# muyeon-jo/POI_recommendation_models

Hardware: AMD Instinct MI355X
Metric: scored (user,POI) pairs/sec full-catalog + top-50, 100k POIs (higher is better)
Workload: dtype fp32-faithful: W1 x products as 6 f16 MFMA products of exact hi/mid/lo fp16 splits (dropped terms <= ~2^-33 relative, below fp32 rounding), fp32 accumulate; all other arithmetic fp32

## Files before the change

### include/nais.h

```cpp
#ifndef NAIS_H_
#define NAIS_H_

#include <stddef.h>
#include <stdint.h>

#ifdef __cplusplus
extern "C" {
#endif

#define NAIS_ABI_VERSION 19

#define NAIS_VARIANT_BASIC 0
#define NAIS_VARIANT_REGION 1
#define NAIS_VARIANT_REGION_DISTANCE 2
#define NAIS_VARIANT_DISTANCE 3

#define NAIS_PRECISION_FP32 0
#define NAIS_PRECISION_FP16X3 1
#define NAIS_PRECISION_FP16X3_PAIRSPLIT 2
#define NAIS_PRECISION_FP16X6 3
#define NAIS_PRECISION_FP16X6_PAIRSPLIT 4

#define NAIS_FLAG_SIGMOID 1

#define NAIS_OK 0
#define NAIS_E_INVALID (-1)
#define NAIS_E_UNSUPPORTED (-2)
#define NAIS_E_HIP (-3)
#define NAIS_E_WORKSPACE (-4)

typedef struct nais_params {
  int32_t variant;
  int32_t embed_dim;
  int32_t item_dim;
  int32_t region_dim;
  int32_t hidden;
  int32_t din;
  int64_t num_pois;
  int64_t num_regions;
  float beta;
  int32_t precision;
  const float* embed_history;
  const float* embed_target;
  const float* embed_region;
  const float* w1;
  const float* b1;
  const float* w2;
  const float* dist_w;
  const float* dist_b;
} nais_params_t;

typedef struct nais_prior {
  double a, b, alpha;
  const double* coords;
} nais_prior_t;

int32_t nais_abi_version(void);

const char* nais_last_error(void);

int32_t nais_forward(const nais_params_t* params,
                     const int64_t* hist, int64_t b, int64_t n, int64_t hist_ld,
                     const int64_t* target,
                     const int64_t* hist_region, int64_t hist_region_ld,
                     const int64_t* target_region,
                     const float* target_lat_long, int64_t latlon_ld,
                     float* out, int32_t* nan_count, int32_t flags, void* stream);

size_t nais_score_topk_workspace_size(const nais_params_t* params, int32_t num_users, int32_t k,
                                      int32_t with_prior);
int32_t nais_score_topk(const nais_params_t* params,
                        const int64_t* indptr, const int64_t* indices,
                        const int32_t* users, int32_t num_users, int32_t k,
                        const int64_t* region_of, const double* coords,
                        const double* latlon_mat, const nais_prior_t* prior,
                        int32_t* out_ids, float* out_scores,
                        int32_t* nan_count, int32_t* short_count,
                        void* workspace, size_t workspace_bytes, void* stream);

int32_t nais_score_catalog(const nais_params_t* params,
                           const int64_t* indptr, const int64_t* indices,
                           const int32_t* users, int32_t num_users,
                           const int64_t* region_of, const double* coords, const double* latlon_mat,
                           float* scores, int64_t score_ld, int32_t* nan_count, void* stream);

int32_t nais_powerlaw_prior(const double* coords, int64_t num_pois, const int64_t* indptr,
                            const int64_t* indices, const int32_t* users, int32_t num_users, double a,
                            double b, double* out, int64_t out_ld, double* out_max, void* stream);

int32_t nais_distance_histogram(const double* coords, const int64_t* indptr, const int64_t* indices,
                                int64_t num_users, uint64_t* hist, int64_t nbins, uint64_t* overflow,
                                void* stream);

int32_t nais_topk_rows(const float* scores, int64_t score_ld, int64_t num_pois, int32_t num_rows,
                       int32_t k, int32_t* out_ids, float* out_scores, int32_t* short_count,
                       void* stream);

int32_t nais_gather_rows(const float* table, int64_t rows, int32_t dim,
                         const int64_t* idx, int64_t m, float* out, void* stream);

size_t nais_pair_rows_workspace_size(int64_t num_pois);
int32_t nais_pair_rows(const int64_t* indptr, const int64_t* indices, const int32_t* users,
                       int32_t num_users, int64_t num_pois, int32_t* rowmap, int64_t* items,
                       int64_t* num_items, void* workspace, size_t workspace_bytes, void* stream);
int32_t nais_pair_table(const nais_params_t* params, const int64_t* items, int64_t num_items,
                        int64_t col0, int64_t cols, const int64_t* region_of,
                        const double* coords, const double* latlon_mat, float* e, float* es,
                        int64_t ld, int32_t* work, void* stream);
int32_t nais_pair_gather(const float* e, const float* es, int64_t ld, const int32_t* rowmap,
                         const int64_t* indptr, const int64_t* indices, const int32_t* users,
                         int32_t num_users, int64_t col0, int64_t cols, float beta, float* scores,
                         int64_t score_ld, int64_t score_col0, int32_t* nan_count, void* stream);
int32_t nais_pair_gather_topk(const float* e, const float* es, int64_t ld, const int32_t* rowmap,
                              const int64_t* indptr, const int64_t* indices, const int32_t* users,
                              int32_t num_users, int64_t col0, int64_t cols, float beta, int32_t k,
                              uint64_t* keys, int32_t* kcount, int32_t* nan_count, int32_t* work,
                              void* stream);
int32_t nais_topk_keys_finish(const uint64_t* keys, const int32_t* kcount, int32_t num_users, int32_t k,
                              int32_t* out_ids, float* out_scores, int32_t* short_count, void* stream);
int32_t nais_pair_table_split(const nais_params_t* params, const int64_t* items, int64_t num_items,
                              int64_t col0, int64_t cols, const int64_t* region_of,
                              const double* coords, const double* latlon_mat, uint32_t* hi,
                              uint32_t* ex, int64_t ld, int32_t* work, void* stream);
int32_t nais_pair_bound_topk(const uint32_t* hi, int64_t ld, const int32_t* rowmap,
                             const int64_t* indptr, const int64_t* indices, const int32_t* users,
                             int32_t num_users, int64_t col0, int64_t cols, float beta, int32_t k,
                             uint64_t* lo_keys, int32_t* lo_count, uint64_t* surv, int32_t* surv_count,
                             int32_t surv_cap, const int32_t* entry_rows, const int64_t* spans,
                             int32_t* work, void* stream);
int32_t nais_pair_refine_topk(const uint32_t* ex, int64_t block_stride,
                              int64_t ld, int64_t block_cols, const int32_t* rowmap,
                              const int64_t* indptr, const int64_t* indices, const int32_t* users,
                              int32_t num_users, int64_t col0, int64_t cols, float beta, int32_t k,
                              const uint64_t* lo_keys, const int32_t* lo_count, const uint64_t* surv,
                              const int32_t* surv_count, int32_t surv_cap, const uint64_t* tau,
                              uint64_t* keys, int32_t* kcount, int32_t* nan_count, int32_t* stats,
                              const int32_t* entry_rows, void* stream);
int32_t nais_pair_table_bound(const nais_params_t* params, const int64_t* items, int64_t num_items,
                              int64_t col0, int64_t cols, const int64_t* region_of,
                              const double* coords, const double* latlon_mat, uint32_t* hi,
                              int64_t ld, void* stream);
int32_t nais_pair_table_bound_queued(const nais_params_t* params, const int64_t* items,
                                     int64_t num_items, int64_t col0, int64_t cols,
                                     const int64_t* region_of, const double* coords,
                                     const double* latlon_mat, uint32_t* hi, int64_t ld,
                                     int32_t* work, void* stream);
int32_t nais_pair_table_bound1_queued(const nais_params_t* params, const int64_t* items,
                                      int64_t num_items, int64_t col0, int64_t cols,
                                      const int64_t* region_of, const double* coords,
                                      const double* latlon_mat, uint32_t* hi, int64_t ld,
                                      int32_t* work, void* stream);
int32_t nais_pair_bound_topk_widened(const uint32_t* hi, int64_t ld, const int32_t* rowmap,
                                     const int64_t* indptr, const int64_t* indices, const int32_t* users,
                                     int32_t num_users, int64_t col0, int64_t cols, float beta, int32_t k,
                                     uint64_t* lo_keys, int32_t* lo_count, uint64_t* surv,
                                     int32_t* surv_count, int32_t surv_cap, const int32_t* entry_rows,
                                     const int64_t* spans, const float* widen, int32_t* work,
                                     void* stream);
int32_t nais_pair_scales(const nais_params_t* params, const int64_t* items, int64_t num_items,
                         int64_t col0, int64_t cols, int64_t block_cols, float* row_scales,
                         float* col_scales, void* stream);
int32_t nais_pair_refine_topk_exact(const nais_params_t* params, const float* row_scales,
                                    const float* col_scales, const int32_t* rowmap, const int64_t* indptr,
                                    const int64_t* indices, const int32_t* users, int32_t num_users,
                                    int64_t col0, int64_t cols, int32_t k, const uint64_t* lo_keys,
                                    const int32_t* lo_count, const uint64_t* surv, const int32_t* surv_count,
                                    int32_t surv_cap, const uint64_t* tau, uint64_t* keys, int32_t* kcount,
                                    int32_t* nan_count, int32_t* stats, const int32_t* entry_rows,
                                    void* stream);
int32_t nais_pair_recompute(const nais_params_t* params, const int64_t* items, int64_t num_items,
                            const float* row_scales, const float* col_scales, int64_t col0, int64_t cols,
                            const int32_t* rows, int64_t num_rows, const int64_t* columns,
                            int64_t num_columns, float* out_e, float* out_es, void* stream);
int32_t nais_pair_prior_table(const double* coords, int64_t num_pois, const int64_t* items,
                              int64_t num_items, int64_t col0, int64_t cols, double a, double b,
                              double* pr, int64_t ld, void* stream);
#define NAIS_PRIOR_FINITE 1
int32_t nais_pair_prior_gather(const double* pr, int64_t ld, const int32_t* rowmap,
                               const int64_t* indptr, const int64_t* indices, const int32_t* users,
                               int32_t num_users, int64_t col0, int64_t cols, double* g, int64_t g_ld,
                               int64_t g_col0, uint64_t* gmax_bits, int32_t flags, void* stream);
int32_t nais_topk_blend_rows(const float* scores, int64_t score_ld, const double* g, int64_t g_ld,
                             const uint64_t* gmax_bits, int64_t num_pois, int32_t num_rows, int32_t k,
                             double alpha, int32_t* out_ids, float* out_scores, int32_t* short_count,
                             void* stream);
int32_t nais_topk_blend_rows_f64(const float* scores, int64_t score_ld, const double* g, int64_t g_ld,
                                 const uint64_t* gmax_bits, int64_t num_pois, int32_t num_rows, int32_t k,
                                 double alpha, int32_t* out_ids, float* out_scores, double* out_blend,
                                 int32_t* short_count, void* stream);
int32_t nais_topk_merge_f64(const double* keys, const int64_t* ids, int32_t num_rows, int32_t m,
                            int32_t k, int64_t* out_ids, float* out_scores, double* out_keys,
                            void* stream);

int32_t nais_stream_create_cu_mask(const uint32_t* cu_mask, uint32_t mask_words, void** stream);
int32_t nais_stream_destroy(void* stream);

int32_t nais_new4_tables(const float* embed_history, const float* embed_target,
                         const float* embed_ingoing, const float* embed_outgoing,
                         int64_t num_pois, int32_t embed_size, const int64_t* near_pois,
                         int32_t num_near, float* ext_history, float* ext_target, void* stream);

int32_t nais_near_attention(const float* query_src, const float* kv_src, int64_t num_pois,
                            int32_t dim, const int64_t* near_pois, int32_t num_near,
                            const float* wq, const float* bq, const float* wk, const float* bk,
                            const float* wv, const float* bv, float scale_dim, float* out,
                            int64_t out_ld, void* stream);
int32_t nais_copy_columns(const float* src, int64_t src_ld, int64_t rows, int32_t dim, float* dst,
                          int64_t dst_ld, int32_t dst_col0, void* stream);

typedef struct nais_dot_tables {
  int32_t embed_dim;
  int64_t num_pois;
  float beta;
  float scale_dim;
  const float* xh;
  const float* xt;
  const float* qt;
  const float* kh;
  const float* vh;
} nais_dot_tables_t;
// ... 194 lines not shown
```

### poi_recommendation_models_amd/_capi.py

```python
from __future__ import annotations

import ctypes
import os

HERE = os.path.dirname(os.path.abspath(__file__))
LIB_NAME = "libnais_hip.so"
LIB_PATH = os.path.join(HERE, LIB_NAME)

ABI_VERSION = 19
PRECISION_FP32, PRECISION_FP16X3, PRECISION_FP16X3_PAIRSPLIT = 0, 1, 2
PRIOR_FINITE = 1
PRECISION_FP16X6, PRECISION_FP16X6_PAIRSPLIT = 3, 4
VARIANT_BASIC, VARIANT_REGION, VARIANT_REGION_DISTANCE, VARIANT_DISTANCE = 0, 1, 2, 3
FLAG_SIGMOID = 1

EXPORTS = ("nais_abi_version", "nais_last_error", "nais_forward", "nais_score_topk_workspace_size",
           "nais_score_topk", "nais_score_catalog", "nais_topk_rows", "nais_powerlaw_prior",
           "nais_distance_histogram", "nais_gather_rows", "nais_train_workspace_size",
           "nais_train_forward", "nais_train_backward", "nais_dropout_mask", "nais_adagrad",
           "nais_adagrad_rows", "nais_train_step_workspace_size", "nais_train_step", "nais_train_step_ex",
           "nais_make_train_batch", "nais_new4_tables", "nais_pair_rows_workspace_size",
           "nais_pair_rows", "nais_pair_table", "nais_pair_gather", "nais_stream_create_cu_mask",
           "nais_stream_destroy", "nais_near_attention", "nais_copy_columns",
           "nais_linear_rows", "nais_dot_forward", "nais_dot_pair_table", "nais_dot_single_fixup",
           "nais_disent_forward", "nais_pair_distances", "nais_train_forward_ex",
           "nais_train_backward_ex", "nais_pair_gather_topk", "nais_topk_keys_finish",
           "nais_pair_prior_table",
           "nais_pair_prior_gather", "nais_topk_blend_rows", "nais_topk_blend_rows_f64",
           "nais_topk_merge_f64", "nais_train_ucache_size", "nais_pair_table_split",
           "nais_pair_bound_topk", "nais_pair_refine_topk", "nais_pair_table_bound",
           "nais_pair_bound_topk_widened", "nais_pair_scales", "nais_pair_refine_topk_exact",
           "nais_pair_recompute", "nais_pair_table_bound_queued", "nais_pair_table_bound1_queued",
           "nais_geoie_table", "nais_geoie_score", "nais_geoie_forward",
           "nais_geoie_make_train_batch", "nais_geoie_train_step_workspace_size",
           "nais_geoie_train_step", "nais_sgd")


class NaisGeoIEParams(ctypes.Structure):
    _fields_ = [("embed_dim", ctypes.c_int32), ("num_users", ctypes.c_int64),
                ("num_pois", ctypes.c_int64), ("a", ctypes.c_float), ("b", ctypes.c_float)] + \
        [(n, ctypes.c_void_p) for n in ("user_pref", "poi_pref", "geo_influence", "geo_suscept")]


class NaisGeoIETrainGrads(ctypes.Structure):
    _fields_ = [(n, ctypes.c_void_p) for n in ("user_pref", "poi_pref", "geo_suscept", "geo_influence")]


class NaisDotTables(ctypes.Structure):
    _fields_ = [("embed_dim", ctypes.c_int32), ("num_pois", ctypes.c_int64), ("beta", ctypes.c_float),
                ("scale_dim", ctypes.c_float), ("xh", ctypes.c_void_p), ("xt", ctypes.c_void_p),
                ("qt", ctypes.c_void_p), ("kh", ctypes.c_void_p), ("vh", ctypes.c_void_p)]


class NaisTrainSide(ctypes.Structure):
    _fields_ = [("hist_region", ctypes.c_void_p), ("target_region", ctypes.c_void_p),
                ("target_lat_long", ctypes.c_void_p), ("latlon_ld", ctypes.c_int64),
                ("ucache", ctypes.c_void_p), ("ucache_bytes", ctypes.c_uint64)]


class NaisTrainGrads(ctypes.Structure):
    _fields_ = [(n, ctypes.c_void_p) for n in ("embed_history", "embed_target", "embed_region", "w1",
                                               "b1", "w2", "dist_w", "dist_b")]


class NaisDisentParams(ctypes.Structure):
    _fields_ = [("embed_dim", ctypes.c_int32), ("hidden", ctypes.c_int32), ("num_pois", ctypes.c_int64),
                ("num_regions", ctypes.c_int64), ("beta", ctypes.c_float)] + \
        [(n, ctypes.c_void_p) for n in ("embed_history", "embed_target", "embed_region", "embed_distance",
                                        "w1", "b1", "w2", "region_w1", "region_b1", "region_w2")]


class NaisParams(ctypes.Structure):
    _fields_ = [
        ("variant", ctypes.c_int32), ("embed_dim", ctypes.c_int32), ("item_dim", ctypes.c_int32),
        ("region_dim", ctypes.c_int32), ("hidden", ctypes.c_int32), ("din", ctypes.c_int32),
        ("num_pois", ctypes.c_int64), ("num_regions", ctypes.c_int64),
        ("beta", ctypes.c_float), ("precision", ctypes.c_int32),
        ("embed_history", ctypes.c_void_p), ("embed_target", ctypes.c_void_p),
        ("embed_region", ctypes.c_void_p), ("w1", ctypes.c_void_p), ("b1", ctypes.c_void_p),
        ("w2", ctypes.c_void_p), ("dist_w", ctypes.c_void_p), ("dist_b", ctypes.c_void_p),
    ]


class NaisPrior(ctypes.Structure):
    _fields_ = [("a", ctypes.c_double), ("b", ctypes.c_double), ("alpha", ctypes.c_double),
                ("coords", ctypes.c_void_p)]


class NaisAdagradState(ctypes.Structure):
    _fields_ = [("lr", ctypes.c_float), ("lr_decay", ctypes.c_float),
                ("weight_decay", ctypes.c_float), ("eps", ctypes.c_float), ("step", ctypes.c_int64)] + \
        [(n, ctypes.c_void_p) for n in ("sum_embed_history", "sum_embed_target", "sum_w1", "sum_b1",
                                        "sum_w2", "grad_embed_history", "grad_embed_target",
                                        "grad_small", "stamp_embed_history", "stamp_embed_target")]


class NaisAdagradSide(ctypes.Structure):
    _fields_ = [(n, ctypes.c_void_p) for n in ("sum_embed_region", "grad_embed_region", "sum_dist_w",
                                               "sum_dist_b", "grad_dist")]


class NaisError(RuntimeError):
    pass


_lib = None


def load(path: str | None = None):
    global _lib
    if _lib is not None and path is None:
        return _lib
    p = path or os.environ.get("NAIS_HIP_LIB", LIB_PATH)
    if not os.path.exists(p):
        raise NaisError(f"{p} not found: build it with `python -c 'import __graft_entry__ as g; g.build()'` "
# ... 48 lines not shown
    lib.nais_train_step.argtypes = [ctypes.POINTER(NaisParams), ctypes.POINTER(NaisAdagradState), vp,
                                    i64, vp, vp, i64, f32, u64, vp, vp, vp, vp, sz, vp]
    lib.nais_train_step_ex.restype = i32
    lib.nais_train_step_ex.argtypes = [ctypes.POINTER(NaisParams), ctypes.POINTER(NaisTrainSide),
                                       ctypes.POINTER(NaisAdagradState), ctypes.POINTER(NaisAdagradSide),
                                       vp, i64, vp, vp, i64, f32, u64, vp, vp, vp, vp, sz, vp]
    lib.nais_make_train_batch.restype = i32
    lib.nais_make_train_batch.argtypes = [vp, vp, i64, i64, i64, i32, u64, vp, vp, vp, vp, vp]
    lib.nais_new4_tables.restype = i32
    lib.nais_new4_tables.argtypes = [vp, vp, vp, vp, i64, i32, vp, i32, vp, vp, vp]
    lib.nais_near_attention.restype = i32
    lib.nais_near_attention.argtypes = [vp, vp, i64, i32, vp, i32, vp, vp, vp, vp, vp, vp,
                                        ctypes.c_float, vp, i64, vp]
    lib.nais_linear_rows.restype = i32
    lib.nais_linear_rows.argtypes = [vp, i64, i64, i32, vp, vp, i32, vp, i64, vp]
    lib.nais_dot_forward.restype = i32
    lib.nais_dot_forward.argtypes = [ctypes.POINTER(NaisDotTables), vp, i64, i64, i64, vp, vp, vp, i32, vp]
    lib.nais_dot_pair_table.restype = i32
    lib.nais_dot_pair_table.argtypes = [ctypes.POINTER(NaisDotTables), vp, i64, i64, i64, vp, vp, i64, vp]
    lib.nais_dot_single_fixup.restype = i32
    lib.nais_dot_single_fixup.argtypes = [ctypes.POINTER(NaisDotTables), vp, vp, vp, i64, i64, i64, vp,
                                          i64, i64, vp]
    lib.nais_train_forward_ex.restype = i32
    lib.nais_train_forward_ex.argtypes = [ctypes.POINTER(NaisParams), ctypes.POINTER(NaisTrainSide), vp, i64,
                                          vp, i64, f32, u64, vp, vp, vp, vp, ctypes.c_size_t, vp]
    lib.nais_train_backward_ex.restype = i32
    lib.nais_train_backward_ex.argtypes = [ctypes.POINTER(NaisParams), ctypes.POINTER(NaisTrainSide), vp,
                                           i64, vp, i64, f32, u64, vp, vp, vp,
                                           ctypes.POINTER(NaisTrainGrads), vp, ctypes.c_size_t, vp]
    lib.nais_disent_forward.restype = i32
    lib.nais_disent_forward.argtypes = [ctypes.POINTER(NaisDisentParams), vp, i64, i64, i64, vp, vp, i64, vp,
                                        vp, i64, vp, vp, i32, vp]
    lib.nais_pair_distances.restype = i32
    lib.nais_pair_distances.argtypes = [vp, vp, i64, vp, i64, vp, vp]
    lib.nais_copy_columns.restype = i32
    lib.nais_copy_columns.argtypes = [vp, i64, i64, i32, vp, i64, i32, vp]
    lib.nais_pair_rows_workspace_size.restype = sz
    lib.nais_pair_rows_workspace_size.argtypes = [i64]
    lib.nais_pair_rows.restype = i32
    lib.nais_pair_rows.argtypes = [vp, vp, vp, i32, i64, vp, vp, vp, vp, sz, vp]
    lib.nais_pair_table.restype = i32
    lib.nais_pair_table.argtypes = [ctypes.POINTER(NaisParams), vp, i64, i64, i64, vp, vp, vp, vp, vp,
                                    i64, vp, vp]
    lib.nais_pair_gather.restype = i32
    lib.nais_pair_gather.argtypes = [vp, vp, i64, vp, vp, vp, vp, i32, i64, i64, f32, vp, i64, i64, vp,
                                     vp]
    lib.nais_pair_gather_topk.restype = i32
    lib.nais_pair_gather_topk.argtypes = [vp, vp, i64, vp, vp, vp, vp, i32, i64, i64, f32, i32, vp, vp, vp,
                                          vp, vp]
    lib.nais_pair_prior_table.restype = i32
    lib.nais_pair_prior_table.argtypes = [vp, i64, vp, i64, i64, i64, f64, f64, vp, i64, vp]
    lib.nais_pair_prior_gather.restype = i32
    lib.nais_pair_prior_gather.argtypes = [vp, i64, vp, vp, vp, vp, i32, i64, i64, vp, i64, i64, vp, i32, vp]
    lib.nais_topk_blend_rows.restype = i32
    lib.nais_topk_blend_rows.argtypes = [vp, i64, vp, i64, vp, i64, i32, i32, f64, vp, vp, vp, vp]
    lib.nais_topk_blend_rows_f64.restype = i32
    lib.nais_topk_blend_rows_f64.argtypes = [vp, i64, vp, i64, vp, i64, i32, i32, f64, vp, vp, vp, vp, vp]
    lib.nais_train_ucache_size.restype = sz
    lib.nais_train_ucache_size.argtypes = [ctypes.POINTER(NaisParams), i64, i64]
    lib.nais_topk_merge_f64.restype = i32
    lib.nais_topk_merge_f64.argtypes = [vp, vp, i32, i32, i32, vp, vp, vp, vp]
    lib.nais_topk_keys_finish.restype = i32
    lib.nais_topk_keys_finish.argtypes = [vp, vp, i32, i32, vp, vp, vp, vp]
    lib.nais_pair_table_split.restype = i32
    lib.nais_pair_table_split.argtypes = [ctypes.POINTER(NaisParams), vp, i64, i64, i64, vp, vp, vp, vp,
                                          vp, i64, vp, vp]
    lib.nais_pair_bound_topk.restype = i32
    lib.nais_pair_bound_topk.argtypes = [vp, i64, vp, vp, vp, vp, i32, i64, i64, f32, i32, vp, vp, vp, vp,
                                         i32, vp, vp, vp, vp]
    lib.nais_pair_refine_topk.restype = i32
    lib.nais_pair_refine_topk.argtypes = [vp, i64, i64, i64, vp, vp, vp, vp, i32, i64, i64, f32, i32,
                                          vp, vp, vp, vp, i32, vp, vp, vp, vp, vp, vp, vp]
    lib.nais_pair_table_bound.restype = i32
    lib.nais_pair_table_bound.argtypes = [ctypes.POINTER(NaisParams), vp, i64, i64, i64, vp, vp, vp, vp,
                                          i64, vp]
    lib.nais_pair_table_bound_queued.restype = i32
    lib.nais_pair_table_bound_queued.argtypes = [ctypes.POINTER(NaisParams), vp, i64, i64, i64, vp, vp, vp,
                                                 vp, i64, vp, vp]
    lib.nais_pair_table_bound1_queued.restype = i32
    lib.nais_pair_table_bound1_queued.argtypes = lib.nais_pair_table_bound_queued.argtypes
    lib.nais_pair_bound_topk_widened.restype = i32
    lib.nais_pair_bound_topk_widened.argtypes = [vp, i64, vp, vp, vp, vp, i32, i64, i64, f32, i32, vp, vp,
                                                 vp, vp, i32, vp, vp, vp, vp, vp]
    lib.nais_pair_scales.restype = i32
    lib.nais_pair_scales.argtypes = [ctypes.POINTER(NaisParams), vp, i64, i64, i64, i64, vp, vp, vp]
    lib.nais_pair_refine_topk_exact.restype = i32
    lib.nais_pair_refine_topk_exact.argtypes = [ctypes.POINTER(NaisParams), vp, vp, vp, vp, vp, vp, i32,
                                                i64, i64, i32, vp, vp, vp, vp, i32, vp, vp, vp, vp, vp,
                                                vp, vp]
    lib.nais_pair_recompute.restype = i32
    lib.nais_pair_recompute.argtypes = [ctypes.POINTER(NaisParams), vp, i64, vp, vp, i64, i64, vp, i64,
                                        vp, i64, vp, vp, vp]
    lib.nais_geoie_table.restype = i32
    lib.nais_geoie_table.argtypes = [vp, vp, i64, vp, i64, i64, i64, f32, f32, vp, i64, vp]
    lib.nais_geoie_score.restype = i32
    lib.nais_geoie_score.argtypes = [ctypes.POINTER(NaisGeoIEParams), vp, vp, vp, i32, vp, vp, i64,
                                     i64, i64, i64, vp, i64, i64, vp, vp]
    lib.nais_geoie_forward.restype = i32
    lib.nais_geoie_forward.argtypes = [ctypes.POINTER(NaisGeoIEParams), vp, vp, vp, i64, i64, i64, vp,
                                       i64, vp, vp]
    lib.nais_geoie_make_train_batch.restype = i32
    lib.nais_geoie_make_train_batch.argtypes = [vp, vp, vp, i64, i64, i64, i32, u64, vp, vp, vp, vp, vp,
                                                vp, vp, i64, vp, vp]
    lib.nais_geoie_train_step_workspace_size.restype = sz
    lib.nais_geoie_train_step_workspace_size.argtypes = [ctypes.POINTER(NaisGeoIEParams), i64, i64]
    lib.nais_geoie_train_step.restype = i32
    lib.nais_geoie_train_step.argtypes = [ctypes.POINTER(NaisGeoIEParams), i64, vp, i64, vp, vp, vp, i64,
                                          vp, i64, f32, f32, vp, vp, i32, vp, vp, vp, vp,
                                          ctypes.POINTER(NaisGeoIETrainGrads), vp, sz, vp]
    lib.nais_sgd.restype = i32
    lib.nais_sgd.argtypes = [vp, vp, i64, i32, f32, f32, vp, i32, i64, vp, vp]
    lib.nais_stream_create_cu_mask.restype = i32
    lib.nais_stream_create_cu_mask.argtypes = [vp, ctypes.c_uint32, ctypes.POINTER(ctypes.c_void_p)]
    lib.nais_stream_destroy.restype = i32
    lib.nais_stream_destroy.argtypes = [vp]
    v = lib.nais_abi_version()
    if v != ABI_VERSION:
        raise NaisError(f"{p}: ABI version {v}, expected {ABI_VERSION}")
    if path is None:
        _lib = lib
    return lib


def check(rc: int, what: str):
    if rc != 0:
        msg = load().nais_last_error().decode(errors="replace")
        raise NaisError(f"{what} failed ({rc}): {msg}")


def ptr(t) -> int | None:
    return None if t is None else t.data_ptr()


def stream_handle(device) -> int:
    import torch
    return torch.cuda.current_stream(device).cuda_stream
```

### poi_recommendation_models_amd/catalog.py

```python
from __future__ import annotations

import ctypes
import os

import numpy as np
import torch

from . import _capi


class DeviceCSR:

    def __init__(self, train_matrix, device):
        X = train_matrix.tocsr() if not hasattr(train_matrix, "indptr") else train_matrix
        if not X.has_sorted_indices:
            X = X.sorted_indices()
        self.shape = X.shape
        self.host_indptr = np.asarray(X.indptr, dtype=np.int64)
        self.host_indices = np.asarray(X.indices, dtype=np.int64)
        self.hist_len = np.diff(self.host_indptr)
        self.indptr = torch.from_numpy(self.host_indptr).to(device)
        self.indices = torch.from_numpy(self.host_indices).to(device)
        self.device = device
        self.key = (id(train_matrix), X.shape, X.nnz)
# ... 92 lines not shown
    if stream is not None:
        ext = torch.cuda.ExternalStream(stream, device=dev)
        cur = torch.cuda.current_stream(dev)
        ext.wait_stream(cur)
        with torch.cuda.stream(ext):
            out = score_topk(model, train_matrix, users, k, region_of, coords, latlon_mat, ordered,
                             None, prior, strategy, _on_caller_stream=True)
        cur.wait_stream(ext)
        for t in out:
            t.record_stream(cur)
        return out
    strategy = strategy or getattr(model, "catalog_strategy", "auto")
    if strategy not in ("auto", "direct", "pairs"):
        raise ValueError(f"unknown strategy {strategy!r}")
    if model._pairs_only:
        if prior is not None:
            raise NotImplementedError(f"{type(model).__name__}: no power-law prior on its catalog path")
        strategy = "pairs"
    if strategy != "direct":
        got = _score_topk_pairs(model, train_matrix, users, k, region_of, coords, latlon_mat,
                                stream, force=strategy == "pairs", prior=prior,
                                no_side_streams=_on_caller_stream)
        if got is not None:
            return got
    csr = device_csr(train_matrix, dev)
    P = model._item_tables()[0].shape[0]
    if csr.shape[1] != P:
        raise ValueError(f"train_matrix has {csr.shape[1]} POIs, model has {P}")
    users = _user_array(users)
    if len(users) == 0:
        return (torch.empty(0, k, dtype=torch.int64, device=dev),
                torch.empty(0, k, dtype=torch.float32, device=dev))
    if np.any(P - csr.hist_len[users] < k):
        raise RuntimeError("selected index k out of range")
    order = lpt_order(users, csr.hist_len, P) if ordered else users
    u_dev = torch.from_numpy(order.astype(np.int32)).to(dev)
    reg, cor, llm = _side_inputs(model, dev, region_of, coords, latlon_mat)
    n = len(order)
    ids = torch.empty(n, k, dtype=torch.int32, device=dev)
    sc = torch.empty(n, k, dtype=torch.float32, device=dev)
    counters = torch.zeros(2, dtype=torch.int32, device=dev)
    lib = _capi.load()
    prm = model._score_params()
    pri, pri_coords = None, None
    if prior is not None:
        pa, pb, alpha, pc = prior
        pri_coords = torch.as_tensor(np.ascontiguousarray(pc, dtype=np.float64)).to(dev)
        prior_flags = _capi.PRIOR_FINITE if _prior_entries_finite(pa, pb) else 0
        pri = _capi.NaisPrior(float(pa), float(pb), float(alpha), pri_coords.data_ptr())
    nbytes = lib.nais_score_topk_workspace_size(prm, n, k, int(prior is not None))
    ws = _workspace(dev, nbytes)
    st = stream if stream is not None else _capi.stream_handle(dev)
    rc = lib.nais_score_topk(prm, csr.indptr.data_ptr(), csr.indices.data_ptr(), u_dev.data_ptr(),
                             n, k, _capi.ptr(reg), _capi.ptr(cor), _capi.ptr(llm),
                             None if pri is None else ctypes.byref(pri),
                             ids.data_ptr(), sc.data_ptr(), counters[0:1].data_ptr(),
                             counters[1:2].data_ptr(), ws.data_ptr(), ws.numel(), st)
    _capi.check(rc, "nais_score_topk")
    model._last_nan = counters[0:1]
    if ordered:
        inv = np.empty(n, dtype=np.int64)
        pos = {int(u): i for i, u in enumerate(order)}
        inv[:] = [pos[int(u)] for u in users]
        inv_t = torch.from_numpy(inv).to(dev)
        ids, sc = ids.index_select(0, inv_t), sc.index_select(0, inv_t)
    return ids.to(torch.int64), sc


PAIR_BLOCK_COLS = 512
PAIR_TABLE_CUS = -1
PAIR_FIRST_TABLE_ALL_CUS = True
PAIR_FUSED_TOPK = True
PAIR_LPT_ORDER = True
PAIR_STRIPE = 256
PAIR_CU_LAYOUT = "contiguous"
PAIR_TABLE_GATHER_FRAC = 0.0
PAIR_TABLE_STREAMS = int(os.environ.get("NAIS_PAIR_TABLE_STREAMS", "2"))
PAIR_WORK_QUEUE = os.environ.get("NAIS_PAIR_WORK_QUEUE", "1") != "0"
PAIR_SPLIT_STEP = 8
X3Q_RATE = 1.10e15
X3Q_GATHER_MARGIN = 1.14
X1Q_RATE = 6.0e14
X1Q_GATHER_MARGIN = 1.34
PAIR_BOUNDED = True
PAIR_ONDEMAND_REFINE = os.environ.get("NAIS_PAIR_ONDEMAND_REFINE", "1") != "0"
PAIR_ONDEMAND_ETA_MAX = 2.0 ** -9
PAIR_ONDEMAND_ONE_PRODUCT = os.environ.get("NAIS_PAIR_ONDEMAND_ONE_PRODUCT", "1") != "0"
PAIR_ONDEMAND_ETA1_MAX = 2.0 ** -7
PAIR_SURV_CAP = 1024
PAIR_SHORT_CHAINS = os.environ.get("NAIS_PAIR_SHORT_CHAINS", "1") != "0"
PAIR_BOUNDED_STRIPE = 512
_masked: dict = {}


def bounded_gather_cu_seconds(entries, NC, users, k):
    launches = np.ceil(NC / PAIR_BOUNDED_STRIPE)
    ins = k * (1.0 + np.log(max(float(NC), float(k)) / k))
    return entries * NC * 4.0 / 90.4e9 + 512e-9 * users * launches + 68e-9 * users * ins


def ondemand_widening(model, products=3):
    eh, et = model._item_tables()
    w1, b1, w2 = model.attn_layer1.weight, model.attn_layer1.bias, model.attn_layer2.weight
    srcs = (eh, et, w1, b1, w2)
    key = tuple((t.data_ptr(), t._version) for t in srcs)
    if products not in (1, 3):
        raise ValueError("products: 1 or 3")
    hit = model.__dict__.get("_widen_cache")
    if hit is not None and hit[0] == key and products in hit[1]:
        return hit[1][products]
    with torch.no_grad():
        f64 = torch.float64
        D = next((w for w in (8, 16, 32, 64, 128) if w >= w1.shape[1]), w1.shape[1])
        HP = 32 if w1.shape[0] <= 32 else 64
        u = 2.0 ** -23
        g = lambda n: n * u / (1.0 - n * u)
        H2 = torch.linalg.vector_norm(eh.to(f64), dim=1).max()
        T2 = torch.linalg.vector_norm(et.to(f64), dim=1).max()
        Hinf, Tinf = eh.abs().max().to(f64), et.abs().max().to(f64)
        Winf = w1.abs().amax(dim=1).to(f64)
        Z = b1.abs().to(f64) + Winf * H2 * T2
        q = D * 2.0 ** -36 * Winf.max() * Hinf * Tinf
        theta = (g(6 * D + 1) + g(3 * D + 1)) * (1 + 2.0 ** -8) + 2.0 ** -23 + 2.0 ** -20
        theta_a = theta
        if products == 1:
            theta_a = ((g(6 * D + 1) + g(D + 1)) * (1 + 2.0 ** -8) + 2.0 ** -23
                       + 2.0 ** -10 * (1 + 2.0 ** -9))
        eta_a = (w2.abs().to(f64).reshape(-1) * (theta_a * Z + q + (HP + 4) * u * 1.01 * Z)).sum()
        eta = eta_a * (1 + eta_a) + 2.0 ** -20
        ds = theta * H2 * T2 + D * 2.0 ** -36 * Hinf * Tinf
        ok = ((Winf.max() * Hinf < 2.0 ** 100) & (Winf.max() * Hinf > 2.0 ** -100) &
              (Tinf < 2.0 ** 100) & (Tinf > 2.0 ** -100))
        both = torch.stack([eta, ds]) * (1 + 2.0 ** -20)
        both = torch.where(ok & torch.isfinite(both).all(), both, torch.full_like(both, float("inf")))
        widen = both.to(torch.float32)
        eta_h, ds_h = (float(v) for v in both.cpu())
    out = (widen, eta_h, ds_h)
    if hit is None or hit[0] != key:
        hit = model.__dict__["_widen_cache"] = (key, {})
    hit[1][products] = out
    return out


def ondemand_form(eta1, eta3):
    if PAIR_ONDEMAND_ONE_PRODUCT and np.isfinite(eta1) and eta1 <= PAIR_ONDEMAND_ETA1_MAX:
        return 1
    if np.isfinite(eta3) and eta3 <= PAIR_ONDEMAND_ETA_MAX:
        return 3
    return None


def _ondemand_shape(model, prm):
    return (prm.variant == _capi.VARIANT_BASIC and prm.precision == _capi.PRECISION_FP16X6
            and prm.embed_dim in (32, 64) and prm.hidden <= 64)


def auto_table_cus(model, J, NC, entries, ncu, prior=False, block_bytes=None, work_queues=True,
                   gather_bytes=8, k=None, users=None, products=None, table_queue=False):
    H, din = model.attn_layer1.weight.shape
    prec = getattr(model, "precision", "fp16x6")
    given = products
    if products is None:
        products = 1 if prec == "fp32" else (6 if prec.startswith("fp16x6") else 3)
    dist = getattr(model, "VARIANT", 0) in (_capi.VARIANT_REGION_DISTANCE, _capi.VARIANT_DISTANCE)
    D = din - 2 if dist else din
    D = next((w for w in (8, 16, 32, 64, 128) if w >= D), D)
    gbytes = entries * NC * float(gather_bytes)
    if prior:
        gbytes *= 2
    xcd = max(1, ncu // 8)
    x6n = (PAIR_WORK_QUEUE and work_queues and products == 6 and D in (32, 64, 128) and H <= 128
           and not prior)
    step = min(PAIR_SPLIT_STEP, xcd) if x6n else xcd
    x3q = (PAIR_WORK_QUEUE and work_queues and table_queue and products == 3 and gather_bytes == 4
           and D in (16, 32, 64, 128) and H <= 128 and not prior and not dist)
    rate = 1.47e15 if x6n else 1.25e15
    if x3q:
        rate = X3Q_RATE
    x1q = (PAIR_WORK_QUEUE and work_queues and table_queue and given == 1 and gather_bytes == 4
           and D in (32, 64) and H <= 64 and not prior and not dist)
    din_k = D + (2 if dist else 0)
    t_tab = J * NC * 2.0 * H * din_k * products / (1.3e14 if products == 1 else rate)
    if x1q:
        t_tab = J * NC * 2.0 * H * din_k / X1Q_RATE
    if x6n and dist:
        t_tab *= 1.0 + 16.0 / (3.0 * D)
    if prior:
        t_tab += J * NC * 1.4e-11
    per_cu = 72e9 if block_bytes is None or block_bytes <= 512e6 else 51e9
    if gather_bytes == 4:
        per_cu = 66e9
        if x6n or x3q or x1q:
            step = 2
        if users and k:
            per_cu = gbytes / bounded_gather_cu_seconds(entries, NC, users, k)
        if x3q:
            per_cu /= X3Q_GATHER_MARGIN
        if x1q:
            per_cu /= X1Q_GATHER_MARGIN
    cap = 7.5e12
    best, best_t = ncu // 2, None
    for n in range((ncu // 4 + step - 1) // step * step, ncu - step + 1, step):
        g_pen = 1.0
        if gather_bytes == 4 and PAIR_CU_LAYOUT == "contiguous" and (ncu - 1) // xcd - n // xcd + 1 <= 2:
            g_pen = 1.04
        t = max(t_tab * ncu / n, gbytes * g_pen / min(cap, (ncu - n) * per_cu))
        if best_t is None or t <= best_t:
            best, best_t = n, t
    return best


def _destroy_masked_streams():
    if not _masked:
        return
    lib = _capi.load()
    for pair in _masked.values():
        for s in pair:
            s.synchronize()
            lib.nais_stream_destroy(s.cuda_stream)
    _masked.clear()


def _masked_streams(dev, table_cus):
    key = (str(dev), table_cus, PAIR_CU_LAYOUT)
    hit = _masked.get(key)
    if hit is not None:
        return hit
    n = torch.cuda.get_device_properties(dev).multi_processor_count
    if PAIR_CU_LAYOUT == "contiguous":
        mine = set(range(table_cus))
    else:
        mine = {int(i * n / table_cus) for i in range(table_cus)}
    words = (n + 31) // 32
    masks = []
    for sel in (mine, set(range(n)) - mine, mine):
        m = (ctypes.c_uint32 * words)()
        for c in sel:
            m[c // 32] |= 1 << (c % 32)
        masks.append(m)
    lib = _capi.load()
    out = []
    with torch.cuda.device(dev):
        for m in masks:
            h = ctypes.c_void_p()
            _capi.check(lib.nais_stream_create_cu_mask(m, words, ctypes.byref(h)), "nais_stream_create_cu_mask")
            out.append(torch.cuda.ExternalStream(h.value, device=dev))
    if not _masked:
        import atexit
        atexit.register(_destroy_masked_streams)
    _masked[key] = tuple(out)
    return _masked[key]


def _score_topk_pairs(model, train_matrix, users, k, region_of, coords, latlon_mat, stream, force,
                      rows_only=False, cols=None, events=None, prior=None, no_side_streams=False,
                      group=None, return_keys=False, tau_group=None):
    dev = model._check_device()
    csr = device_csr(train_matrix, dev)
    P = model._item_tables()[0].shape[0]
    if csr.shape[1] != P:
        raise ValueError(f"train_matrix has {csr.shape[1]} POIs, model has {P}")
    c0_all, c1_all = cols if cols is not None else (0, P)
    NC = c1_all - c0_all
    users = _user_array(users)
    n = len(users)
    if n == 0 or NC <= 0:
        return None
    if cols is None and np.any(P - csr.hist_len[users] < k):
        raise RuntimeError("selected index k out of range")
    lib = _capi.load()
    st = stream if stream is not None else _capi.stream_handle(dev)
    torch_stream = torch.cuda.current_stream(dev)
    order = None
    if PAIR_LPT_ORDER and not rows_only and n > 1:
        order = np.argsort(-csr.hist_len[users], kind="stable")
    up = np.concatenate([users if order is None else users[order],
                         np.argsort(order, kind="stable") if order is not None else np.zeros(0, np.int64)])
    up_dev = torch.from_numpy(up.astype(np.int32)).pin_memory().to(dev, non_blocking=True)
    u_all = up_dev[:n]
    reg, cor, llm = _side_inputs(model, dev, region_of, coords, latlon_mat)
    prm = model._score_params()
    rowmap = torch.empty(P, dtype=torch.int32, device=dev)
    items = torch.empty(P, dtype=torch.int64, device=dev)
    cnt = torch.zeros(1, dtype=torch.int64, device=dev)
    ws = _workspace(dev, lib.nais_pair_rows_workspace_size(P))

    def timed(kind, fn, launches=1):
        if events is None:
            return fn()
        e0, e1 = torch.cuda.Event(enable_timing=True), torch.cuda.Event(enable_timing=True)
        e0.record(torch_stream)
        r = fn()
        e1.record(torch_stream)
        events.append((kind, e0, e1, launches))
        return r

    def rows(u_dev, m):
        _capi.check(lib.nais_pair_rows(csr.indptr.data_ptr(), csr.indices.data_ptr(), u_dev.data_ptr(),
                                       m, P, rowmap.data_ptr(), items.data_ptr(), cnt.data_ptr(),
                                       ws.data_ptr(), ws.numel(), st), "nais_pair_rows")
        return int(cnt.item())
    J = rows(u_all, n)
    entries = int(csr.hist_len[users].sum())
    if not force and (J == 0 or entries < PAIR_MIN_SHARING * J):
        return None
    usable = usable_device_bytes(dev)
    budget = int(usable * PAIR_MEMORY_FRACTION)
    from .model import _NAISDevice
    if prior is not None and (rows_only or model._pairs_only):
        raise NotImplementedError("the pairs route blends the prior over the rows of NAIS models only")
    if prior is not None and cols is not None and (c0_all, c1_all) != (0, P) and group is None:
        raise ValueError("a prior over a column shard needs the process group of the other shards "
                         "(the normaliser max G runs over the whole catalog)")
    fused = (PAIR_FUSED_TOPK and not rows_only and J > 0 and k <= 256 and prior is None
             and type(model)._pair_fixup is _NAISDevice._pair_fixup)
    bounded_ok = fused and PAIR_BOUNDED and type(model)._pair_table is _NAISDevice._pair_table
    ond = None
    ond_products = 3
    if bounded_ok and PAIR_ONDEMAND_REFINE and _ondemand_shape(model, prm):
        widen, eta, ds = ondemand_widening(model)
        widen1, eta1, _ = ondemand_widening(model, products=1)
        ond_products = ondemand_form(eta1, eta)
        if ond_products is not None:
            ond = widen1 if ond_products == 1 else widen
        if events is not None:
            events.extend((("ondemand_eta", None, None, eta), ("ondemand_delta_s", None, None, ds),
                           ("ondemand_eta_accepted", None, None, ond is not None),
                           ("ondemand_eta1", None, None, eta1),
                           ("ondemand_products", None, None, ond_products if ond is not None else 0)))
    if prior is not None:
        pa, pb, alpha, pc = prior
        pri_coords = torch.as_tensor(np.ascontiguousarray(pc, dtype=np.float64)).to(dev)
        prior_flags = _capi.PRIOR_FINITE if _prior_entries_finite(pa, pb) else 0
    pr_of = {}

    wq_slots = torch.zeros(8, dtype=torch.int32, device=dev) if PAIR_WORK_QUEUE else None
    wq_of = {}
    wq_on = [False]

    def wq(stream_):
        if wq_slots is None or not wq_on[0]:
            return None
        h = int(stream_ or 0)
        if h not in wq_of:
            if len(wq_of) >= wq_slots.numel():
                raise RuntimeError("pairs route: more streams than work-queue counters")
            wq_of[h] = wq_slots.data_ptr() + 4 * len(wq_of)
        return wq_of[h]

    def table(tab, c0, w, stream_):
        if isinstance(tab, tuple) and len(tab) == 1:
            if ond_products == 1:
                _capi.check(lib.nais_pair_table_bound1_queued(
                    prm, items.data_ptr(), J, c0, w, _capi.ptr(reg), _capi.ptr(cor), _capi.ptr(llm),
                    tab[0].data_ptr(), ld, wq(stream_), stream_), "nais_pair_table_bound1_queued")
                return
            _capi.check(lib.nais_pair_table_bound_queued(
                prm, items.data_ptr(), J, c0, w, _capi.ptr(reg), _capi.ptr(cor), _capi.ptr(llm),
                tab[0].data_ptr(), ld, wq(stream_), stream_), "nais_pair_table_bound_queued")
            return
        if isinstance(tab, tuple):
            _capi.check(lib.nais_pair_table_split(prm, items.data_ptr(), J, c0, w, _capi.ptr(reg),
                                                  _capi.ptr(cor), _capi.ptr(llm), tab[0].data_ptr(),
                                                  tab[1].data_ptr(), ld, wq(stream_), stream_),
                        "nais_pair_table_split")
            return
        model._pair_table(lib, prm, items, J, c0, w, reg, cor, llm, tab[0].data_ptr(),
                          tab[1].data_ptr(), ld, stream_, work=wq(stream_))
        if prior is not None:
            _capi.check(lib.nais_pair_prior_table(pri_coords.data_ptr(), P, items.data_ptr(), J, c0, w,
                                                  float(pa), float(pb), pr_of[id(tab)].data_ptr(), ld,
                                                  stream_), "nais_pair_prior_table")
    row_bytes = 4 * NC + (8 * NC if prior is not None else 0)
    per_pass = n if (rows_only or fused) else max(1, min(n, (budget // 2) // row_bytes))
    if prior is not None and group is not None:
        from .sharding import agree_min
        per_pass = agree_min(per_pass, dev, group)
    if events is not None:
        npass = (n + per_pass - 1) // per_pass
        events.extend((name, None, None, v) for name, v in (
            ("passes", npass), ("users_per_pass", per_pass), ("distinct_rows", J),
            ("usable_bytes", usable), ("budget_bytes", budget)))
    keys_out = torch.empty(n, k, dtype=torch.float64, device=dev) if return_keys else None
    ids_out = torch.empty(n, k, dtype=torch.int32, device=dev)
    sc_out = torch.empty(n, k, dtype=torch.float32, device=dev)
    counters = torch.zeros(2, dtype=torch.int32, device=dev)
    for b0 in range(0, n, per_pass):
        m = min(per_pass, n - b0)
        u_dev = u_all[b0:b0 + m]
        if b0 > 0 or m < n:
            J = rows(u_dev, m)
        bnd = [False]
        ondm = [False]

        def gather_launches(w):
            stripe = PAIR_BOUNDED_STRIPE if bnd[0] else PAIR_STRIPE
            return (w + stripe - 1) // stripe if fused else 1
        if fused:
            keys = torch.empty(m, k, dtype=torch.int64, device=dev)
            kcount = torch.zeros(m, dtype=torch.int32, device=dev)

            def gather(tab, c0, w, stream_, a=0, b=None):
                b = m if b is None else b
                if b <= a:
                    return
                if bnd[0]:
                    _capi.check(lib.nais_pair_bound_topk_widened(
                        tab[0].data_ptr(), ld, rowmap.data_ptr(), csr.indptr.data_ptr(), csr.indices.data_ptr(),
                        u_dev.data_ptr() + 4 * a, b - a, c0, w, float(model.beta), k,
                        lokeys.data_ptr() + 8 * k * a, locount.data_ptr() + 4 * a,
                        surv.data_ptr() + 8 * PAIR_SURV_CAP * a, scount.data_ptr() + 4 * a, PAIR_SURV_CAP,
                        _capi.ptr(erows), spans.data_ptr() + 16 * a if spans is not None else None,
                        ond.data_ptr() if ondm[0] else None, wq(stream_), stream_),
                        "nais_pair_bound_topk_widened")
                    return
                _capi.check(lib.nais_pair_gather_topk(
                    tab[0].data_ptr(), tab[1].data_ptr(), ld, rowmap.data_ptr(), csr.indptr.data_ptr(),
                    csr.indices.data_ptr(), u_dev.data_ptr() + 4 * a, b - a, c0, w, float(model.beta), k,
                    keys.data_ptr() + 8 * k * a, kcount.data_ptr() + 4 * a, counters[0:1].data_ptr(),
                    wq(stream_), stream_), "nais_pair_gather_topk")
        else:
            scores = torch.empty(m, NC, dtype=torch.float32, device=dev)
            if prior is not None:
                G = torch.empty(m, NC, dtype=torch.float64, device=dev)
                gmax = torch.zeros(m, dtype=torch.int64, device=dev)

            def gather(tab, c0, w, stream_, a=0, b=None):
                _capi.check(lib.nais_pair_gather(
                    tab[0].data_ptr(), tab[1].data_ptr(), ld, rowmap.data_ptr(), csr.indptr.data_ptr(),
                    csr.indices.data_ptr(), u_dev.data_ptr(), m, c0, w, float(model.beta),
                    scores.data_ptr(), NC, c0_all, counters[0:1].data_ptr(), stream_), "nais_pair_gather")
                if prior is not None:
                    _capi.check(lib.nais_pair_prior_gather(
                        pr_of[id(tab)].data_ptr(), ld, rowmap.data_ptr(), csr.indptr.data_ptr(),
                        csr.indices.data_ptr(), u_dev.data_ptr(), m, c0, w, G.data_ptr(), NC, c0_all,
                        gmax.data_ptr(), prior_flags, stream_), "nais_pair_prior_gather")
        if J > 0:
            W = min(PAIR_BLOCK_COLS, (budget // 4) // ((16 if prior is not None else 8) * J))
            W = int(min(NC, max(256, W // 256 * 256)))
            ld = (W + 3) // 4 * 4
            blocks = list(range(c0_all, c1_all, W))
            bnd[0] = bounded_ok and (len(blocks) * 3 * J * ld * 4 + m * (PAIR_SURV_CAP + k) * 8
                                     <= budget)
            lists = m * (PAIR_SURV_CAP + 2 * k) * 8
            nring = max(1, PAIR_TABLE_STREAMS) + 1
            ondm[0] = (ond is not None and nring * J * ld * 4 + lists + entries * 4 + m * 24
                       + (2 * J + NC) * 4 <= budget)
            if tau_group is not None and bounded_ok:
                from .sharding import agree_min
                bnd[0] = bool(agree_min(int(bnd[0]), dev, tau_group))
                if ond is not None:
                    ondm[0] = bool(agree_min(int(ondm[0]), dev, tau_group))
            bnd[0] = bnd[0] or ondm[0]
            if events is not None:
                events.append(("pair_route", None, None, "ondemand" if ondm[0] else
                               ("split16" if bnd[0] else "exact")))
            if bnd[0]:
                if ondm[0]:
                    ring = [torch.empty(J, ld, dtype=torch.int32, device=dev) for _ in range(nring)]
                    ring_done = [None] * nring
                    rowsc = torch.empty(max(J, 1), 2, dtype=torch.float32, device=dev)
                    colsc = torch.empty(NC, dtype=torch.float32, device=dev)
                    arena = ()
                else:
                    arena = (torch.empty(len(blocks), J, ld, dtype=torch.int32, device=dev),
                             torch.empty(len(blocks), J, 2 * ld, dtype=torch.int32, device=dev))
                    ring = []
                lokeys = torch.empty(m, k, dtype=torch.int64, device=dev)
                locount = torch.zeros(m, dtype=torch.int32, device=dev)
                surv = torch.empty(m, PAIR_SURV_CAP, dtype=torch.int64, device=dev)
                scount = torch.zeros(m, dtype=torch.int32, device=dev)
                erows = spans = None
                if PAIR_SHORT_CHAINS:
                    erows = rowmap.index_select(0, csr.indices)
                    hb_ = csr.indptr.index_select(0, u_dev.to(torch.int64))
                    spans = torch.stack([hb_, csr.indptr.index_select(0, u_dev.to(torch.int64) + 1) - hb_],
                                        1).contiguous()
                if events is not None:
                    events.append(("bounded", None, None, 1))
            ncu = torch.cuda.get_device_properties(dev).multi_processor_count
            wq_both = fused and type(model)._pair_table is _NAISDevice._pair_table
            table_cus = (auto_table_cus(model, J, NC, entries, ncu, prior is not None,
                                        J * ld * (4 if ondm[0] else 8),
                                        work_queues=wq_both, gather_bytes=4 if bnd[0] else 8, k=k,
                                        users=m, products=ond_products if ondm[0] else None,
                                        table_queue=ondm[0])
                         if PAIR_TABLE_CUS < 0 else PAIR_TABLE_CUS)
            wq_on[0] = table_cus % max(1, ncu // 8) != 0 or (ondm[0] and wq_both)
            if events is not None:
                events.append(("table_cus", None, None, table_cus))
                events.append(("block_cols", None, None, W))
            overlap = (0 < table_cus < ncu and len(blocks) > 1 and stream is None
                       and not no_side_streams)
            tabs = ([] if bnd[0] else [torch.empty(2, J, ld, dtype=torch.float32, device=dev)
                                       for _ in range(2 if overlap else 1)])
            if prior is not None:
                pr_of.update({id(t): torch.empty(J, ld, dtype=torch.float64, device=dev) for t in tabs})
            if overlap:
                ts, gs, ts2 = _masked_streams(dev, table_cus)
                tss = (ts, ts2) if PAIR_TABLE_STREAMS > 1 else (ts,)
                first_all = PAIR_FIRST_TABLE_ALL_CUS
                if first_all:
                    w0 = min(W, c1_all - blocks[0])
                    tab0 = ((ring[0],) if ondm[0] else (arena[0][0], arena[1][0])) if bnd[0] else tabs[0]
                    timed("table", lambda: table(tab0, blocks[0], w0, st))
                for t_ in tss:
                    t_.wait_stream(torch_stream)
                gs.wait_stream(torch_stream)
                done_g = [None, None]
                done_tail = None
                m1 = m
                if fused and PAIR_TABLE_GATHER_FRAC > 0 and m > 1:
                    hl = csr.hist_len[up[b0:b0 + m]].astype(np.float64)
                    tail = np.cumsum(hl[::-1])[::-1]
                    m1 = int(np.searchsorted(-tail, -PAIR_TABLE_GATHER_FRAC * hl.sum(), side="left"))
                    m1 = min(max(m1, 1), m)
                if events is not None:
                    share = float(csr.hist_len[up[b0:b0 + m1]].sum()) / max(1.0, float(csr.hist_len[up[b0:b0 + m]].sum()))
                    events.append(("gather_share", None, None, share))
            for b, c0 in enumerate(blocks):
                w = min(W, c1_all - c0)
                tab = (((ring[b % len(ring)],) if ondm[0] else (arena[0][b], arena[1][b])) if bnd[0]
                       else tabs[b % len(tabs)])
                if overlap:
                    tsb = tss[b % len(tss)]
                    if done_g[b % 2] is not None and not bnd[0]:
                        tsb.wait_event(done_g[b % 2])
                    if ondm[0] and ring_done[b % len(ring)] is not None:
                        tsb.wait_event(ring_done[b % len(ring)])
                    if not (b == 0 and first_all):
                        e_t0, e_t1 = torch.cuda.Event(enable_timing=True), torch.cuda.Event(enable_timing=True)
                        e_t0.record(tsb)
                        table(tab, c0, w, tsb.cuda_stream)
                        e_t1.record(tsb)
                        gs.wait_event(e_t1)
                        if events is not None:
                            events.append(("table", e_t0, e_t1, 1))
                    e_g0, e_g1 = torch.cuda.Event(enable_timing=True), torch.cuda.Event(enable_timing=True)
                    e_g0.record(gs)
                    gather(tab, c0, w, gs.cuda_stream, 0, m1)
                    e_g1.record(gs)
                    done_g[b % 2] = e_g1
                    if ondm[0]:
                        ring_done[b % len(ring)] = e_g1
                    if events is not None:
                        events.append(("gather", e_g0, e_g1, gather_launches(w)))
                    if m1 < m:
                        if done_tail is not None and len(tss) > 1:
                            tsb.wait_event(done_tail)
                        gather(tab, c0, w, tsb.cuda_stream, m1, m)
                        done_tail = torch.cuda.Event()
                        done_tail.record(tsb)
                    continue
                timed("table", lambda: table(tab, c0, w, st))
                timed("gather", lambda: gather(tab, c0, w, st), gather_launches(w))
            if overlap:
                torch_stream.wait_stream(gs)
                for t_ in tss:
                    torch_stream.wait_stream(t_)
                for t in [*tabs, *pr_of.values(), *([wq_slots] if wq_slots is not None else []),
                          *((*arena, *ring, lokeys, locount, surv, scount,
                             *((erows, spans) if erows is not None else ())) if bnd[0] else ())]:
                    for t_ in (*tss, gs):
                        t.record_stream(t_)
            if bnd[0]:
                stats = torch.zeros(2, dtype=torch.int32, device=dev)
                tau_g = None
                if tau_group is not None:
                    from .sharding import global_kth_keys
# ... 106 lines not shown
```

### poi_recommendation_models_amd/csrc/nais_kernels.hip

```cpp
#include <hip/hip_runtime.h>

#include <stdint.h>

#include <algorithm>
#include <cmath>
#include <cstdlib>
#include <type_traits>
#include <string>

#include "nais.h"
#include "nais_internal.h"
#include "nais_geo.h"
#include "nais_fp16x6.h"

typedef float floatx16 __attribute__((ext_vector_type(16)));

namespace {

constexpr int WAVES = 8;
constexpr int THREADS = WAVES * 64;
constexpr int CAND_PER_BLOCK = WAVES * 32;
constexpr int JC = 64;
constexpr int TOPK_THREADS = 1024;
constexpr int MAX_K = 1024;
constexpr int MAX_BATCH_USERS = 512;
constexpr int PAIR_GROUP_ITEMS = 128;

struct DevParams {
  const float* eh;
  const float* et;
  const float* er;
  const float* w1;
  const float* b1;
  const float* w2;
  const float* wd;
  const float* bd;
  int64_t P;
  int32_t item_dim, region_dim, H, din;
  float beta;
};

struct TableOut {
  float* e = nullptr;
  float* es = nullptr;
  int64_t ld = 0, col0 = 0, cols = 0, nitems = 0;
  int32_t gi = 0;
  int32_t* work = nullptr;
  int32_t ngroups = 0, ntiles = 0;
  uint32_t sel_e = NAIS_SEL_E;
  int32_t ex = 0;
};
__device__ __forceinline__ void tab_put(const TableOut& t, int64_t row, int64_t x, float e, float es) {
  const int64_t o = row * t.ld + x;
  const uint32_t eb = __float_as_uint(e), sb = __float_as_uint(es);
  t.e[o] = __uint_as_float(__builtin_amdgcn_perm(sb, eb, t.sel_e));
  if (t.ex) {
    reinterpret_cast<float2*>(t.es)[o] = make_float2(e, es);
  } else if (t.es) {
    t.es[o] = es;
  }
}

__device__ __forceinline__ int cat_user_slot() { return blockIdx.y; }
__device__ __forceinline__ int cat_tile() { return blockIdx.x; }
inline dim3 table_grid(const TableOut& t, int ngroups, int cand_per_block = CAND_PER_BLOCK) {
  return dim3((unsigned)((t.cols + cand_per_block - 1) / cand_per_block), (unsigned)ngroups);
}
inline dim3 cat_grid(int64_t P, int nb, int cand_per_block) {
  return dim3((unsigned)((P + cand_per_block - 1) / cand_per_block), (unsigned)nb);
}

template <int VAR>
struct VarT {
  static constexpr bool REGION = VAR == NAIS_VARIANT_REGION || VAR == NAIS_VARIANT_REGION_DISTANCE;
  static constexpr bool DIST = VAR == NAIS_VARIANT_REGION_DISTANCE || VAR == NAIS_VARIANT_DISTANCE;
  static constexpr float DSCALE = VAR == NAIS_VARIANT_DISTANCE ? 1000.f : 100.f;
};

__device__ __forceinline__ floatx16 mfma32(float a, float b, floatx16 c) {
  return __builtin_amdgcn_mfma_f32_32x32x2f32(a, b, c, 0, 0, 0);
}

__device__ __forceinline__ float sigmoidf_ref(float x) { return 1.0f / (1.0f + expf(-x)); }

template <int DH, int HB, bool DIST>
struct Consts {
  static constexpr int A4 = HB * (DH / 4) * 64;
  static constexpr int ADIST = DIST ? HB * 64 : 0;
  static constexpr int EPI = 2 * 2 * HB * 16;
  static constexpr size_t BYTES = size_t(A4) * 16 + size_t(ADIST) * 4 + size_t(EPI) * 4;
};

__device__ __forceinline__ int acc_row(int hb, int r, int hh) {
  return hb * 32 + (r & 3) + 8 * (r >> 2) + 4 * hh;
}

template <int DH, int HB, bool DIST>
__device__ void stage_consts(const DevParams& p, float4* Aimg, float* Adist, float* Eimg, int tid) {
  using C = Consts<DH, HB, DIST>;
  constexpr int D = 2 * DH;
  for (int f = tid; f < C::A4; f += THREADS) {
    const int ln = f & 63, q = (f >> 6) % (DH / 4), hb = (f >> 6) / (DH / 4);
    const int i = hb * 32 + (ln & 31), k0 = (ln >> 5) * DH + 4 * q;
    float4 v = make_float4(0.f, 0.f, 0.f, 0.f);
    if (i < p.H) {
      const float* w = p.w1 + (int64_t)i * p.din + k0;
      v = make_float4(w[0], w[1], w[2], w[3]);
    }
    Aimg[f] = v;
  }
  if (DIST) {
    for (int f = tid; f < C::ADIST; f += THREADS) {
      const int ln = f & 63, hb = f >> 6, i = hb * 32 + (ln & 31);
      Adist[f] = (i < p.H) ? p.w1[(int64_t)i * p.din + D + (ln >> 5)] : 0.f;
    }
  }
  for (int f = tid; f < C::EPI; f += THREADS) {
    const int which = f / (2 * HB * 16), rem = f % (2 * HB * 16);
    const int hh = rem / (HB * 16), hr = rem % (HB * 16), hb = hr / 16, r = hr % 16;
    const int i = acc_row(hb, r, hh);
    Eimg[f] = (i < p.H) ? (which == 0 ? p.b1[i] : p.w2[i]) : 0.f;
  }
}

template <int DH, int HB, bool DIST, typename HPtr, typename EpiT>
__device__ __forceinline__ void item_step(const float4 (&t4)[DH / 4], HPtr hrow,
                                          const float4* __restrict__ Aimg,
                                          const float* __restrict__ Adist, const EpiT& epi,
                                          float distf, int lane, float& a_out, float& s_out) {
  constexpr int HS = HB > 4 ? 4 : HB;
  float sd = 0.f, ap = 0.f;
#pragma unroll 1
  for (int h0 = 0; h0 < HB; h0 += HS) {
// ... 254 lines not shown
                                      : p.et + tgt * p.item_dim + (REGION ? 0 : hh * DH);
#pragma unroll
    for (int q = 0; q < DH / 4; ++q) t4[q] = reinterpret_cast<const float4*>(src)[q];
  }
  const int64_t* hrow_ids = hist + rr * hist_ld;
  DistW dw{0.f, 0.f, 0.f};
  if (DIST) dw = load_distw<VAR>(p, hh);
  auto row_ptr = [&](int64_t j) -> const float* {
    const int64_t item = hrow_ids[j];
    if (REGION && hh) return p.er + hist_region[rr * hreg_ld + j] * p.region_dim;
    return p.eh + item * p.item_dim + (REGION ? 0 : hh * DH);
  };

  Epi<HB, (HB <= 2 && DH <= 32)> epi;
  __syncthreads();
  epi.load(Eimg, hh);

  float S = 0.f, N = 0.f;
  constexpr bool PREFETCH = DH <= 32;
  float4 hcur[DH / 4];
  if (PREFETCH && n > 0) {
    const float* hp = row_ptr(0);
#pragma unroll
    for (int q = 0; q < DH / 4; ++q) hcur[q] = reinterpret_cast<const float4*>(hp)[q];
  }
  for (int64_t j = 0; j < n; ++j) {
    float4 hnext[DH / 4];
    if (!PREFETCH) {
      const float* hp = row_ptr(j);
#pragma unroll
      for (int q = 0; q < DH / 4; ++q) hcur[q] = reinterpret_cast<const float4*>(hp)[q];
    } else if (j + 1 < n) {
      const float* hp = row_ptr(j + 1);
#pragma unroll
      for (int q = 0; q < DH / 4; ++q) hnext[q] = reinterpret_cast<const float4*>(hp)[q];
    }
    float distf = 0.f;
    if (DIST) {
      const float* ll = latlon + rr * ll_ld + 2 * j;
      distf = dist_feature(dw, ll[0], ll[1]);
    }
    float a, s;
    item_step<DH, HB, DIST>(t4, reinterpret_cast<const float*>(hcur), Aimg, Adist, epi, distf,
                            lane, a, s);
    const bool keep = hrow_ids[j] != tgt;
    const float e = expf(a) * (keep ? 1.f : 0.f);
    S += e;
    N += mul_rn(e, s);
    if (PREFETCH && j + 1 < n) {
#pragma unroll
      for (int q = 0; q < DH / 4; ++q) hcur[q] = hnext[q];
    }
  }
  const float logit = finish_logit(S, N, p.beta, n == 0);
  const bool isnan_ = logit != logit;
  float o = (flags & NAIS_FLAG_SIGMOID) ? sigmoidf_ref(logit) : logit;
  if (valid && hh == 0) out[r] = o;
  if (nan_count) {
    const unsigned long long m = __ballot(valid && hh == 0 && isnan_);
    if (lane == 0 && m) atomicAdd(nan_count, (int32_t)__popcll(m));
  }
}


__device__ __forceinline__ floatx16 mfma16(half8 a, half8 b, floatx16 c) {
  return __builtin_amdgcn_mfma_f32_32x32x16_f16(a, b, c, 0, 0, 0);
}

template <int NPC>
__device__ __forceinline__ floatx16 mfma_pieces(const half8 (&a)[NPC], const half8 (&b)[NPC], floatx16 c) {
  if constexpr (NPC == 2) {
    c = mfma16(a[1], b[0], c);
    c = mfma16(a[0], b[1], c);
    c = mfma16(a[0], b[0], c);
  } else {
    c = mfma16(a[2], b[0], c);
    c = mfma16(a[1], b[1], c);
    c = mfma16(a[0], b[2], c);
    c = mfma16(a[1], b[0], c);
    c = mfma16(a[0], b[1], c);
    c = mfma16(a[0], b[0], c);
  }
  return c;
}

__device__ __forceinline__ float2 lane_halves(float v) {
  const auto r = __builtin_amdgcn_permlane32_swap(__float_as_uint(v), __float_as_uint(v), false, false);
  return make_float2(__uint_as_float(r[0]), __uint_as_float(r[1]));
}

template <int NW>
__device__ float block_max_n(float v, float* red) {
#pragma unroll
  for (int o = 32; o > 0; o >>= 1) v = fmaxf(v, __shfl_xor(v, o));
  const int wave = threadIdx.x >> 6, lane = threadIdx.x & 63;
  __syncthreads();
  if (lane == 0) red[wave] = v;
  __syncthreads();
  float m = red[0];
#pragma unroll
  for (int w = 1; w < NW; ++w) m = fmaxf(m, red[w]);
  return m;
}

__device__ float block_max(float v, float* red) {
#pragma unroll
  for (int o = 32; o > 0; o >>= 1) v = fmaxf(v, __shfl_xor(v, o));
  const int wave = threadIdx.x >> 6, lane = threadIdx.x & 63;
  __syncthreads();
  if (lane == 0) red[wave] = v;
  __syncthreads();
  float m = red[0];
#pragma unroll
  for (int w = 1; w < WAVES; ++w) m = fmaxf(m, red[w]);
  return m;
}

template <int DH, int HB, bool DIST, int NPC = 2>
struct Consts16 {
  static constexpr int KS = DH / 8;
  static constexpr int A16 = HB * KS * NPC * 64;
  static constexpr int ADIST = DIST ? HB * 64 : 0;
  static constexpr int EPI = 2 * 2 * HB * 16;
  static constexpr size_t BYTES = size_t(A16) * 16 + size_t(ADIST) * 4 + size_t(EPI) * 4 + 64;
};

template <int HB, bool REGS>
struct Epi16;
template <int HB>
struct Epi16<HB, true> {
  float bs[HB * 16], ws[HB * 16];
  __device__ __forceinline__ void rescale(const float* Eimg, int hh, float S, float invS) {
#pragma unroll
    for (int i = 0; i < HB * 16; ++i) {
      bs[i] = Eimg[hh * HB * 16 + i] * S;
      ws[i] = Eimg[2 * HB * 16 + hh * HB * 16 + i] * invS;
    }
  }
  __device__ __forceinline__ float init(int i) const { return bs[i]; }
  __device__ __forceinline__ float term(int i, float acc, float) const {
    return ws[i] * relu_bits(acc);
  }
};
template <int HB>
struct Epi16<HB, false> {
  const float* pb;
  const float* pw;
  __device__ __forceinline__ void rescale(const float* Eimg, int hh, float, float) {
    pb = Eimg + hh * HB * 16;
    pw = Eimg + 2 * HB * 16 + hh * HB * 16;
  }
  __device__ __forceinline__ float init(int) const { return 0.f; }
  __device__ __forceinline__ float term(int i, float acc, float invS) const {
    return pw[i] * relu_bits(__builtin_fmaf(acc, invS, pb[i]));
  }
};

template <int HB>
struct Epi16L {
  const float* pb;
  const float* pw;
  __device__ __forceinline__ void rescale(const float* mine, int hh, float, float) {
    pb = mine + hh * HB * 16;
    pw = mine + 2 * HB * 16 + hh * HB * 16;
  }
  __device__ __forceinline__ float init(int i) const { return pb[i]; }
// ... 182 lines not shown
        x[7] = tv[8 * s + 7] * h1.w;
#pragma unroll
        for (int e = 0; e < 8; ++e) sd += x[e];
        half8 xp[NPC];
        split_pieces<NPC>(x, xp);
#pragma unroll
        for (int hb = 0; hb < HB; ++hb) {
          half8 ap_[NPC];
#pragma unroll
          for (int q = 0; q < NPC; ++q) ap_[q] = *reinterpret_cast<const half8*>(&ac[hb][q]);
          acc[hb] = mfma_pieces<NPC>(ap_, xp, acc[hb]);
        }
        __builtin_amdgcn_sched_barrier(0);
      }
      if (DIST) {
        float ll0, ll1;
        if (coords) {
          ll0 = (float)fabs(clat - hco[2 * jj]);
          ll1 = (float)fabs(clon - hco[2 * jj + 1]);
        } else {
          ll0 = (float)llrow[2 * (int64_t)hid[jj]];
          ll1 = (float)llrow[2 * (int64_t)hid[jj] + 1];
        }
        const float fs = dist_feature(dw, ll0, ll1) * St;
#pragma unroll
        for (int hb = 0; hb < HB; ++hb) acc[hb] = mfma32(Adist[hb * 64 + lane], fs, acc[hb]);
      }
      float ap = 0.f;
#pragma unroll
      for (int hb = 0; hb < HB; ++hb)
#pragma unroll
        for (int r = 0; r < 16; ++r) ap += epi.term(hb * 16 + r, acc[hb][r], invS);
      const float a = ap + __shfl_xor(ap, 32);
      const float sv = (sd + __shfl_xor(sd, 32)) * invSt;
      const bool keep = hid[jj] != (int32_t)c;
      const float e = expf(a) * (keep ? 1.f : 0.f);
      if (tab.e) {
        if (valid && hh == 0) {
          tab_put(tab, hbeg + j0 + jj, c - tab.col0, e, e * sv);
        }
        continue;
      }
      in_hist |= !keep;
      S += e;
      N += mul_rn(e, sv);
    }
  }
  if (tab.e) return;

  const float logit = finish_logit(S, N, p.beta, hlen == 0);
  const bool isnan_ = logit != logit;
  float sc = sigmoidf_ref(logit);
  if (isnan_) sc = __builtin_nanf("");
  if (in_hist) sc = -1.f;
  if (valid && hh == 0) scores[(int64_t)cat_user_slot() * score_ld + c] = sc;
  if (nan_count) {
    const unsigned long long m = __ballot(valid && hh == 0 && !in_hist && isnan_);
    if (lane == 0 && m) atomicAdd(nan_count, (int32_t)__popcll(m));
  }
}

template <int DH, int HB, bool DIST, int NW = WAVES, int NPC = 2, int NPA = NPC>
struct CfgB {
  static constexpr int D = 2 * DH;
  static constexpr int KS = DH / 8;
  static constexpr int NE = HB * KS * 64;
  static constexpr int IB = NE * 16 * NPA;
  static constexpr int G = IB <= 16384 ? 4 : (IB <= 32768 ? 2 : 1);
  static constexpr int JCB =
      (NPC == 3) ? 32 : (2 * G * (IB / NPA * NPC) + 64 * D * 4 > 140 * 1024 ? 32 : 64);
  static constexpr int EPT = (NE + NW * 64 - 1) / (NW * 64);
  static constexpr int ADIST = DIST ? HB * 64 : 0;
  static constexpr int EPI = 2 * 2 * HB * 16;
  static constexpr bool PIPE = HB <= 2 && DH <= 32;
  static constexpr bool EREGS = PIPE && NPC == 2;
  static constexpr bool WLDS = PIPE && !EREGS;
  static constexpr int ESCL = WLDS ? NW * EPI : 0;
  static constexpr size_t REST = size_t(ADIST) * 4 + size_t(EPI) * 4 + size_t(ESCL) * 4 + 64 +
                                 size_t(JCB) * D * 4 + size_t(JCB) * 4 + (DIST ? size_t(JCB) * 16 : 0);
  static constexpr size_t BYTES = size_t(2) * G * IB + REST;
  static_assert(!PIPE || G % 2 == 0, "the pipelined steps alternate two accumulator sets per item");
};

template <int DH, int HB, int VAR, int NW, int NPC, bool QUEUE = false, bool ONE = false>
__global__ void __launch_bounds__(NW * 64, NW >= 8 ? 1 : 8 / NW)
catalog_score_x3b_kernel(DevParams p, const int64_t* __restrict__ indptr,
                         const int64_t* __restrict__ indices, const int32_t* __restrict__ users,
                         const int64_t* __restrict__ region_of, const double* __restrict__ coords,
                         const double* __restrict__ latlon_mat, float* __restrict__ scores,
                         int64_t score_ld, int32_t* __restrict__ nan_count, TableOut tab) {
  constexpr bool REGION = VarT<VAR>::REGION;
  constexpr bool DIST = VarT<VAR>::DIST;
  constexpr int NPA = ONE ? 1 : NPC;
  using C = CfgB<DH, HB, DIST, NW, NPC, NPA>;
  constexpr int D = C::D, KS = C::KS, NE = C::NE, G = C::G, JCB = C::JCB, EPT = C::EPT;
  constexpr int THREADS = NW * 64, CAND_PER_BLOCK = NW * 32;
  constexpr bool PIPE = C::PIPE;
  static_assert(!ONE || (NPC == 2 && PIPE && !DIST),
                "one-product logits: the pipelined fp16x3 shapes, no distance inputs");
  constexpr bool SMF = JCB == 32;
  extern __shared__ __attribute__((aligned(16))) char smem[];
  uint4* ring = reinterpret_cast<uint4*>(smem);
  float* Adist = reinterpret_cast<float*>(ring + 2 * G * NPA * NE);
  float* Eimg = Adist + C::ADIST;
  float* Escl = Eimg + C::EPI;
  float* red = Escl + C::ESCL;
  float* hrows = red + 16;
  int32_t* hid = reinterpret_cast<int32_t*>(hrows + JCB * D);
  double* hco = reinterpret_cast<double*>(hid + JCB);

  const int tid = threadIdx.x, lane = tid & 63, wave = tid >> 6, hh = lane >> 5;
  int32_t* wi_sh = reinterpret_cast<int32_t*>(red + 15);
  static_assert(NW < 16, "the work item's LDS word sits behind the block reductions' slots");

  float wv[EPT][8];
  float wmax = 0.f;
#pragma unroll
  for (int q = 0; q < EPT; ++q) {
    const int e = tid + q * THREADS;
    const int ln = e & 63, s = (e >> 6) % KS, hb = (e >> 6) / KS;
    const int i = hb * 32 + (ln & 31), k0 = (ln >> 5) * DH + 8 * s;
#pragma unroll
    for (int x = 0; x < 8; ++x) {
      wv[q][x] = (e < NE && i < p.H) ? p.w1[(int64_t)i * p.din + k0 + x] : 0.f;
      wmax = fmaxf(wmax, fabsf(wv[q][x]));
    }
  }
  const float Wmax = block_max_n<NW>(wmax, red);
  if (DIST) {
    for (int f = tid; f < C::ADIST; f += THREADS) {
      const int ln = f & 63, hb = f >> 6, i = hb * 32 + (ln & 31);
      Adist[f] = (i < p.H) ? p.w1[(int64_t)i * p.din + D + (ln >> 5)] : 0.f;
    }
  }
  for (int f = tid; f < C::EPI; f += THREADS) {
    const int which = f / (2 * HB * 16), rem = f % (2 * HB * 16);
    const int hh2 = rem / (HB * 16), hr = rem % (HB * 16), hb = hr / 16, r = hr % 16;
    const int i = acc_row(hb, r, hh2);
    Eimg[f] = (i < p.H) ? (which == 0 ? p.b1[i] : p.w2[i]) : 0.f;
  }

  DistW dw{0.f, 0.f, 0.f};
  if (DIST) dw = load_distw<VAR>(p, hh);
  float SAcur = 1.f;

  static_assert(!QUEUE || !DIST, "the work queue covers the variants without distance inputs");
  int64_t wslot = cat_user_slot(), wtile = cat_tile(), cur_tile = -1;
  int64_t c = 0;
  bool valid = false;
  float tv[DH];
  half8 tb[KS][NPC];
  float St = 1.f, invSt = 1.f;
  double clat = 0.0, clon = 0.0;
  const double* llrow = nullptr;
  do {
  if constexpr (QUEUE) {
    __syncthreads();
    if (tid == 0) *wi_sh = atomicAdd(tab.work, 1);
    __syncthreads();
    const int64_t wi = *wi_sh;
    if (wi >= (int64_t)tab.ngroups * tab.ntiles) break;
    wtile = wi / tab.ngroups;
    wslot = wi % tab.ngroups;
  }
  int64_t hbeg, hlen;
  if (tab.e) {
    hbeg = wslot * tab.gi;
    hlen = std::min<int64_t>(tab.gi, tab.nitems - hbeg);
  } else {
    const int64_t u = users[wslot];
    hbeg = indptr[u];
    hlen = indptr[u + 1] - hbeg;
  }
  if (!QUEUE || wtile != cur_tile) {
    cur_tile = wtile;
    c = tab.col0 + wtile * CAND_PER_BLOCK + wave * 32 + (lane & 31);
    valid = c < p.P && (!tab.e || c < tab.col0 + tab.cols);
    const int64_t cc = valid ? c : p.P - 1;
    {
      const float* src = (REGION && hh) ? p.er + region_of[cc] * p.region_dim
                                        : p.et + cc * p.item_dim + (REGION ? 0 : hh * DH);
#pragma unroll
// ... 12 lines not shown
    if constexpr (C::WLDS) {
#pragma unroll
      for (int o = 16; o > 0; o >>= 1) tmax = fmaxf(tmax, __shfl_xor(tmax, o));
    }
    St = pow2_scale(tmax);
    invSt = 1.f / St;
#pragma unroll
    for (int s = 0; s < KS; ++s) {
      float x[8];
#pragma unroll
      for (int e = 0; e < 8; ++e) {
        tv[8 * s + e] *= St;
        x[e] = tv[8 * s + e];
      }
      split_pieces<NPC>(x, tb[s]);
    }
    if (DIST) {
      if (coords) {
        clat = coords[2 * cc];
        clon = coords[2 * cc + 1];
      } else {
        llrow = latlon_mat + cc * p.P * 2;
      }
    }
  }

  float S = 0.f, N = 0.f;
  bool in_hist = false;
  std::conditional_t<C::WLDS, Epi16L<HB>, Epi16<HB, C::EREGS>> epi;

  auto build = [&](int jj, int grp, int it) {
    const float* hr = hrows + jj * D;
    uint4* dst = ring + ((grp * G + it) * NPA) * NE;
#pragma unroll
    for (int q = 0; q < EPT; ++q) {
      const int e = tid + q * THREADS;
      if (e < NE) {
        const int ln = e & 63, s = (e >> 6) % KS;
        const int k0 = (ln >> 5) * DH + 8 * s;
        const float4 h0 = *reinterpret_cast<const float4*>(hr + k0);
        const float4 h1 = *reinterpret_cast<const float4*>(hr + k0 + 4);
        float a[8];
        a[0] = wv[q][0] * h0.x;
        a[1] = wv[q][1] * h0.y;
        a[2] = wv[q][2] * h0.z;
        a[3] = wv[q][3] * h0.w;
        a[4] = wv[q][4] * h1.x;
        a[5] = wv[q][5] * h1.y;
        a[6] = wv[q][6] * h1.z;
        a[7] = wv[q][7] * h1.w;
        if constexpr (ONE) {
          half8 hi;
#pragma unroll
          for (int x = 0; x < 8; ++x) hi[x] = (_Float16)a[x];
          dst[e] = *reinterpret_cast<const uint4*>(&hi);
        } else {
          half8 pc[NPC];
          split_pieces<NPC>(a, pc);
#pragma unroll
          for (int q2 = 0; q2 < NPC; ++q2) dst[q2 * NE + e] = *reinterpret_cast<const uint4*>(&pc[q2]);
        }
      }
    }
  };

  float Sacc = 1.f, invS = 1.f;
  int64_t j0 = 0;
  floatx16 sacc;
  float invShSt = 1.f;

  auto tail = [&](int pj, float ap, float sd, bool live) {
    const float2 aph = lane_halves(ap);
    const float a = aph.x + aph.y;
    float sv;
    if (SMF) {
      const float2 sh2 = lane_halves(sacc[((pj >> 3) << 2) | (pj & 3)]);
      sv = (((pj >> 2) & 1) ? sh2.y : sh2.x) * invShSt;
    } else {
      const float2 sdh = lane_halves(sd);
      sv = (sdh.x + sdh.y) * invSt;
    }
    const bool keep = hid[pj] != (int32_t)c;
    const float e = expf(a) * (keep ? 1.f : 0.f);
    if (live) {
      if (tab.e) {
        if (valid && hh == 0) {
          tab_put(tab, hbeg + j0 + pj, c - tab.col0, e, e * sv);
        }
      } else {
        in_hist |= !keep;
        S += e;
        N += mul_rn(e, sv);
      }
    }
    };

  auto step = [&](auto do_mma, auto do_epi, const uint4* src, floatx16 (&accN)[HB],
                  const floatx16 (&accP)[HB], int cur, int prev, bool live) {
    constexpr bool MMA = decltype(do_mma)::value;
    constexpr bool EPIL = decltype(do_epi)::value;
    constexpr int NV = HB * 16;
    constexpr int VPS = (NV + KS - 1) / KS;
    constexpr int QPS = (DH / 4 + KS - 1) / KS;
    const int pj = live ? prev : 0;
    const float* hr = hrows + pj * D + hh * DH;
    float sd = 0.f, ap = 0.f;
    if (MMA) {
#pragma unroll
      for (int hb = 0; hb < HB; ++hb)
#pragma unroll
        for (int r = 0; r < 16; ++r) accN[hb][r] = epi.init(hb * 16 + r);
    }
#pragma unroll
    for (int s = 0; s < KS; ++s) {
      if (MMA) {
#pragma unroll
        for (int hb = 0; hb < HB; ++hb) {
          half8 ap_[NPA];
#pragma unroll
          for (int q = 0; q < NPA; ++q) {
            const uint4 u4 = src[q * NE + (hb * KS + s) * 64 + lane];
            ap_[q] = *reinterpret_cast<const half8*>(&u4);
          }
          if constexpr (ONE) accN[hb] = mfma16(ap_[0], tb[s][0], accN[hb]);
          else accN[hb] = mfma_pieces<NPC>(ap_, tb[s], accN[hb]);
        }
      }
      if constexpr (EPIL) {
#pragma unroll
        for (int v = s * VPS; v < (s + 1) * VPS && v < NV; ++v)
          ap += epi.term(v, accP[v / 16][v % 16], invS);
      }
      if (EPIL && !SMF) {
#pragma unroll
        for (int q = s * QPS; q < (s + 1) * QPS && q < DH / 4; ++q) {
          const float4 hv = *reinterpret_cast<const float4*>(hr + 4 * q);
          sd = __builtin_fmaf(tv[4 * q], hv.x, sd);
          sd = __builtin_fmaf(tv[4 * q + 1], hv.y, sd);
          sd = __builtin_fmaf(tv[4 * q + 2], hv.z, sd);
          sd = __builtin_fmaf(tv[4 * q + 3], hv.w, sd);
        }
      }
    }
    if (DIST && MMA) {
      float ll0, ll1;
      if (coords) {
        ll0 = (float)fabs(clat - hco[2 * cur]);
        ll1 = (float)fabs(clon - hco[2 * cur + 1]);
      } else {
        ll0 = (float)llrow[2 * (int64_t)hid[cur]];
        ll1 = (float)llrow[2 * (int64_t)hid[cur] + 1];
      }
      const float fs = dist_feature(dw, ll0, ll1) * Sacc;
#pragma unroll
      for (int hb = 0; hb < HB; ++hb) accN[hb] = mfma32(Adist[hb * 64 + lane], fs, accN[hb]);
    }
    if constexpr (EPIL) tail(pj, ap, sd, live);
  };

  auto step_wide = [&](const uint4* src, int cur) {
    constexpr int HS = HB < 2 ? HB : 2;
    float ap = 0.f;
#pragma unroll 1
    for (int h0 = 0; h0 < HB; h0 += HS) {
      floatx16 acc[HS];
#pragma unroll
// ... 1375 lines not shown
int launch_catalog_x3b(const DevParams& d, const int64_t* indptr, const int64_t* indices,
                       const int32_t* users, int nb, const int64_t* region_of, const double* coords,
                       const double* latlon_mat, float* scores, int64_t ld, int32_t* nan_count,
                       hipStream_t stream, const TableOut& tab = TableOut{}) {
  if constexpr (NPC == 3 && (DH == 16 || DH == 32 || DH == 64)) {
    constexpr int D = 2 * DH;
    constexpr int MB = HB <= 2 ? 2 * HB : 4;
    constexpr int NHU = HB <= 2 ? 1 : HB / 2;
    using CN = CfgN<D, MB, NHU, VarT<VAR>::DIST>;
    const size_t lds = CN::BYTES;
    auto kern = catalog_score_x6n_kernel<D, MB, NHU, VAR>;
    static bool attr_set = false;
    if (!attr_set) {
      (void)hipFuncSetAttribute(reinterpret_cast<const void*>(kern),
                                hipFuncAttributeMaxDynamicSharedMemorySize, (int)lds);
      attr_set = true;
    }
    dim3 grid = tab.e ? table_grid(tab, nb, CN::CPB) : cat_grid(d.P, nb, CN::CPB);
    TableOut t = tab;
    if (t.e && t.work) {
      t.ngroups = (int32_t)grid.y;
      t.ntiles = (int32_t)grid.x;
      const int ncu = nais_internal_stream_cus(stream);
      if (ncu <= 0) return fail(NAIS_E_HIP, "device attributes");
      grid = dim3((unsigned)std::min<int64_t>((int64_t)grid.x * grid.y, ncu), 1, 1);
      if (hipMemsetAsync(t.work, 0, sizeof(int32_t), stream) != hipSuccess)
        return fail(NAIS_E_HIP, "hipMemsetAsync(work)");
    } else {
      t.work = nullptr;
    }
    hipLaunchKernelGGL(kern, grid, dim3(CN::THREADS), lds, stream, d, indptr, indices, users,
                       region_of, coords, latlon_mat, scores, ld, nan_count, t);
    return check_launch("catalog_score_x6n_kernel");
  } else if constexpr (HB > 4) {
    return fail(NAIS_E_UNSUPPORTED, "hidden > 128: the catalog kernels take it at precision fp16x6 "
                                    "with embed_dim 32, 64 or 128");
  } else if constexpr (DH % 8 != 0) {
    return launch_catalog<DH, HB, VAR>(d, indptr, indices, users, nb, region_of, coords, latlon_mat,
                                       scores, ld, nan_count, stream, tab);
  } else if constexpr ((VarT<VAR>::DIST && !CfgB<DH, HB, true, WAVES, NPC>::PIPE) ||
                       CfgB<DH, HB, false, WAVES, NPC>::BYTES > kLdsBytes) {
    return launch_catalog_x3<DH, HB, VAR, NPC>(d, indptr, indices, users, nb, region_of, coords,
                                               latlon_mat, scores, ld, nan_count, stream, tab);
  } else {
    constexpr int NW = WAVES;
    const size_t lds = CfgB<DH, HB, VarT<VAR>::DIST, NW, NPC>::BYTES;
    auto kern = catalog_score_x3b_kernel<DH, HB, VAR, NW, NPC>;
    static bool attr_set = false;
    if (!attr_set) {
      (void)hipFuncSetAttribute(reinterpret_cast<const void*>(kern),
                                hipFuncAttributeMaxDynamicSharedMemorySize, (int)lds);
      attr_set = true;
    }
    dim3 grid = tab.e ? table_grid(tab, nb, NW * 32) : cat_grid(d.P, nb, NW * 32);
    TableOut t = tab;
    if constexpr (!VarT<VAR>::DIST) {
      if (t.e && t.work) {
        t.ngroups = (int32_t)grid.y;
        t.ntiles = (int32_t)grid.x;
        auto kq = catalog_score_x3b_kernel<DH, HB, VAR, NW, NPC, true>;
        static bool attr_set_q = false;
        if (!attr_set_q) {
          (void)hipFuncSetAttribute(reinterpret_cast<const void*>(kq),
                                    hipFuncAttributeMaxDynamicSharedMemorySize, (int)lds);
          attr_set_q = true;
        }
        const int ncu = nais_internal_stream_cus(stream);
        if (ncu <= 0) return fail(NAIS_E_HIP, "device attributes");
        grid = dim3((unsigned)std::min<int64_t>((int64_t)grid.x * grid.y, ncu), 1, 1);
        if (hipMemsetAsync(t.work, 0, sizeof(int32_t), stream) != hipSuccess)
          return fail(NAIS_E_HIP, "hipMemsetAsync(work)");
        hipLaunchKernelGGL(kq, grid, dim3(NW * 64), lds, stream, d, indptr, indices, users, region_of,
                           coords, latlon_mat, scores, ld, nan_count, t);
        return check_launch("catalog_score_x3b_kernel (queue)");
      }
    }
    t.work = nullptr;
    hipLaunchKernelGGL(kern, grid, dim3(NW * 64), lds, stream, d, indptr, indices, users, region_of,
                       coords, latlon_mat, scores, ld, nan_count, t);
    return check_launch("catalog_score_x3b_kernel");
  }
}

template <int DH, int HB>
int launch_x3b_one(const DevParams& d, const int64_t* indices, int ng, hipStream_t stream,
                   const TableOut& tab) {
  constexpr int NW = WAVES, VAR = NAIS_VARIANT_BASIC;
  const size_t lds = CfgB<DH, HB, false, NW, 2, 1>::BYTES;
  auto kern = catalog_score_x3b_kernel<DH, HB, VAR, NW, 2, false, true>;
  auto kq = catalog_score_x3b_kernel<DH, HB, VAR, NW, 2, true, true>;
  static bool attr_set = false;
  if (!attr_set) {
    (void)hipFuncSetAttribute(reinterpret_cast<const void*>(kern),
                              hipFuncAttributeMaxDynamicSharedMemorySize, (int)lds);
    (void)hipFuncSetAttribute(reinterpret_cast<const void*>(kq),
                              hipFuncAttributeMaxDynamicSharedMemorySize, (int)lds);
    attr_set = true;
  }
  dim3 grid = table_grid(tab, ng, NW * 32);
  TableOut t = tab;
  if (t.work) {
    t.ngroups = (int32_t)grid.y;
    t.ntiles = (int32_t)grid.x;
    const int ncu = nais_internal_stream_cus(stream);
    if (ncu <= 0) return fail(NAIS_E_HIP, "device attributes");
    grid = dim3((unsigned)std::min<int64_t>((int64_t)grid.x * grid.y, ncu), 1, 1);
    if (hipMemsetAsync(t.work, 0, sizeof(int32_t), stream) != hipSuccess)
      return fail(NAIS_E_HIP, "hipMemsetAsync(work)");
    hipLaunchKernelGGL(kq, grid, dim3(NW * 64), lds, stream, d, nullptr, indices, nullptr, nullptr,
                       nullptr, nullptr, nullptr, 0, nullptr, t);
    return check_launch("catalog_score_x3b_kernel (one product, queue)");
  }
  hipLaunchKernelGGL(kern, grid, dim3(NW * 64), lds, stream, d, nullptr, indices, nullptr, nullptr,
                     nullptr, nullptr, nullptr, 0, nullptr, t);
  return check_launch("catalog_score_x3b_kernel (one product)");
}

template <int DH, int HB, int VAR>
int launch_catalog_x6b(const DevParams& d, const int64_t* indptr, const int64_t* indices,
                       const int32_t* users, int nb, const int64_t* region_of, const double* coords,
                       const double* latlon_mat, float* scores, int64_t ld, int32_t* nan_count,
                       hipStream_t stream, const TableOut& tab = TableOut{}) {
  return launch_catalog_x3b<DH, HB, VAR, 3>(d, indptr, indices, users, nb, region_of, coords,
                                            latlon_mat, scores, ld, nan_count, stream, tab);
}
template <int DH, int HB, int VAR>
int launch_catalog_x6(const DevParams& d, const int64_t* indptr, const int64_t* indices,
                      const int32_t* users, int nb, const int64_t* region_of, const double* coords,
                      const double* latlon_mat, float* scores, int64_t ld, int32_t* nan_count,
                      hipStream_t stream, const TableOut& tab = TableOut{}) {
  return launch_catalog_x3<DH, HB, VAR, 3>(d, indptr, indices, users, nb, region_of, coords,
                                           latlon_mat, scores, ld, nan_count, stream, tab);
}

template <int DH, int HB, int VAR>
int launch_forward(const DevParams& d, const int64_t* hist, int64_t b, int64_t n, int64_t hist_ld,
                   const int64_t* target, const int64_t* hreg, int64_t hreg_ld, const int64_t* treg,
                   const float* latlon, int64_t ll_ld, float* out, int32_t* nan_count, int32_t flags,
                   hipStream_t stream) {
  constexpr bool DIST = VarT<VAR>::DIST;
  const size_t lds = Consts<DH, HB, DIST>::BYTES;
  auto kern = forward_kernel<DH, HB, VAR>;
  static bool attr_set = false;
  if (!attr_set) {
    (void)hipFuncSetAttribute(reinterpret_cast<const void*>(kern),
                        hipFuncAttributeMaxDynamicSharedMemorySize, (int)lds);
    attr_set = true;
  }
  dim3 grid((unsigned)((b + CAND_PER_BLOCK - 1) / CAND_PER_BLOCK));
  hipLaunchKernelGGL(kern, grid, dim3(THREADS), lds, stream, d, hist, b, n, hist_ld, target, hreg,
                     hreg_ld, treg, latlon, ll_ld, out, nan_count, flags);
  return check_launch("forward_kernel");
}

#define NAIS_DISPATCH(FN, DH_, HB_, VAR_, ...)                                   \
  do {                                                                            \
    switch (VAR_) {                                                               \
      case 0: NAIS_DISPATCH_DH(FN, DH_, HB_, 0, __VA_ARGS__); break;              \
      case 1: NAIS_DISPATCH_DH(FN, DH_, HB_, 1, __VA_ARGS__); break;              \
      case 2: NAIS_DISPATCH_DH(FN, DH_, HB_, 2, __VA_ARGS__); break;              \
      default: NAIS_DISPATCH_DH(FN, DH_, HB_, 3, __VA_ARGS__); break;             \
    }                                                                             \
  } while (0)
#define NAIS_DISPATCH_DH(FN, DH_, HB_, V, ...)                                   \
  switch (DH_) {                                                                  \
    case 4: NAIS_DISPATCH_HB(FN, 4, HB_, V, __VA_ARGS__); break;                  \
    case 8: NAIS_DISPATCH_HB(FN, 8, HB_, V, __VA_ARGS__); break;                  \
    case 16: NAIS_DISPATCH_HB(FN, 16, HB_, V, __VA_ARGS__); break;                \
    case 32: NAIS_DISPATCH_HB(FN, 32, HB_, V, __VA_ARGS__); break;                \
    default: NAIS_DISPATCH_HB(FN, 64, HB_, V, __VA_ARGS__); break;                \
  }
#define NAIS_DISPATCH_HB(FN, DH, HB_, V, ...)                                    \
  switch (HB_) {                                                                  \
// ... 87 lines not shown
  if (with_prior) bytes += (size_t)(nb * ld * 8 + round_up(nb, 64) * 8);
  return bytes;
}

int32_t nais_score_topk(const nais_params_t* params, const int64_t* indptr, const int64_t* indices,
                        const int32_t* users, int32_t num_users, int32_t k,
                        const int64_t* region_of, const double* coords,
                        const double* latlon_mat, const nais_prior_t* prior,
                        int32_t* out_ids, float* out_scores, int32_t* nan_count,
                        int32_t* short_count, void* workspace, size_t workspace_bytes,
                        void* stream) {
  Shape sh;
  int rc = validate(params, &sh);
  if (rc) return rc;
  if (num_users < 0) return fail(NAIS_E_INVALID, "num_users < 0");
  if (num_users == 0) return NAIS_OK;
  if (k <= 0 || k > MAX_K) return fail(NAIS_E_UNSUPPORTED, "k must be in [1, 1024]");
  if (!indptr || !indices || !users || !out_ids || !out_scores)
    return fail(NAIS_E_INVALID, "missing indptr/indices/users/outputs");
  if ((params->variant == NAIS_VARIANT_REGION || params->variant == NAIS_VARIANT_REGION_DISTANCE) &&
      !region_of)
    return fail(NAIS_E_INVALID, "region variants need region_of");
  if ((params->variant == NAIS_VARIANT_REGION_DISTANCE || params->variant == NAIS_VARIANT_DISTANCE) &&
      !coords && !latlon_mat)
    return fail(NAIS_E_INVALID, "region_distance needs coords or latlon_mat");
  if (prior && !prior->coords) return fail(NAIS_E_INVALID, "prior needs coords");
  const size_t need = nais_score_topk_workspace_size(params, num_users, k, prior != nullptr);
  if (!workspace || workspace_bytes < need) return fail(NAIS_E_WORKSPACE, "workspace too small");
  hipStream_t st = reinterpret_cast<hipStream_t>(stream);
  DevParams d;
  rc = to_dev(params, &d);
  if (rc) return rc;
  float* scores = reinterpret_cast<float*>(workspace);
  const int64_t ld = round_up(params->num_pois, 64);
  for (int32_t u0 = 0; u0 < num_users; u0 += MAX_BATCH_USERS) {
    const int nb = std::min<int32_t>(MAX_BATCH_USERS, num_users - u0);
    if (sh.gen_cat)
      rc = nais_gx_catalog(params, indptr, indices, users + u0, nb, nullptr, 0, 0, 0, region_of,
                           coords, latlon_mat, scores, ld, nan_count, nullptr, nullptr, 0, st);
    else if (params->precision == NAIS_PRECISION_FP16X6)
      NAIS_DISPATCH(launch_catalog_x6b, sh.DH, sh.HB, params->variant, d, indptr, indices, users + u0,
                    nb, region_of, coords, latlon_mat, scores, ld, nan_count, st);
    else if (params->precision == NAIS_PRECISION_FP16X6_PAIRSPLIT)
      NAIS_DISPATCH(launch_catalog_x6, sh.DH, sh.HB, params->variant, d, indptr, indices, users + u0,
                    nb, region_of, coords, latlon_mat, scores, ld, nan_count, st);
    else if (params->precision == NAIS_PRECISION_FP16X3)
      NAIS_DISPATCH(launch_catalog_x3b, sh.DH, sh.HB, params->variant, d, indptr, indices, users + u0,
                    nb, region_of, coords, latlon_mat, scores, ld, nan_count, st);
    else if (params->precision == NAIS_PRECISION_FP16X3_PAIRSPLIT)
      NAIS_DISPATCH(launch_catalog_x3, sh.DH, sh.HB, params->variant, d, indptr, indices, users + u0,
                    nb, region_of, coords, latlon_mat, scores, ld, nan_count, st);
    else
      NAIS_DISPATCH(launch_catalog, sh.DH, sh.HB, params->variant, d, indptr, indices, users + u0, nb,
                    region_of, coords, latlon_mat, scores, ld, nan_count, st);
    if (rc) return rc;
    if (!prior) {
      hipLaunchKernelGGL(topk_kernel, dim3(nb), dim3(TOPK_THREADS), 0, st, scores, ld,
                         params->num_pois, k, out_ids + (int64_t)u0 * k,
                         out_scores + (int64_t)u0 * k, short_count);
      rc = check_launch("topk_kernel");
      if (rc) return rc;
    } else {
      const int64_t nbmax = std::min<int64_t>(num_users, MAX_BATCH_USERS);
      double* G = reinterpret_cast<double*>(scores + nbmax * ld);
      unsigned long long* gmax = reinterpret_cast<unsigned long long*>(G + nbmax * ld);
      rc = launch_prior(prior->coords, params->num_pois, indptr, indices, users + u0, nb, prior->a,
                        prior->b, G, ld, gmax, st);
      if (rc) return rc;
      hipLaunchKernelGGL(topk_blend_kernel, dim3(nb), dim3(TOPK_THREADS), 0, st, scores, ld, G, ld,
                         gmax, params->num_pois, k, (float)(1.0 - prior->alpha), prior->alpha,
                         out_ids + (int64_t)u0 * k, out_scores + (int64_t)u0 * k, short_count,
                         (double*)nullptr);
      rc = check_launch("topk_blend_kernel");
      if (rc) return rc;
    }
  }
  return NAIS_OK;
}

namespace {
int32_t pair_table_impl(const nais_params_t* params, const int64_t* items, int64_t num_items,
                        int64_t col0, int64_t cols, const int64_t* region_of, const double* coords,
                        const double* latlon_mat, float* e, float* es, int64_t ld, int32_t* work,
                        void* stream, bool split = false, bool bound = false, bool one = false) {
  Shape sh;
  int rc = validate(params, &sh);
  if (rc) return rc;
  if (num_items < 0 || col0 < 0 || cols < 0 || col0 + cols > params->num_pois)
    return fail(NAIS_E_INVALID, "bad item count or column range");
  if (num_items == 0 || cols == 0) return NAIS_OK;
  if (!items || !e || (!es && !bound)) return fail(NAIS_E_INVALID, "missing pointer");
  if (ld < cols) return fail(NAIS_E_INVALID, "ld < cols");
  if ((params->variant == NAIS_VARIANT_REGION || params->variant == NAIS_VARIANT_REGION_DISTANCE) &&
      !region_of)
    return fail(NAIS_E_INVALID, "region variants need region_of");
  if ((params->variant == NAIS_VARIANT_REGION_DISTANCE || params->variant == NAIS_VARIANT_DISTANCE) &&
      !coords && !latlon_mat)
    return fail(NAIS_E_INVALID, "distance variants need coords or latlon_mat");
  hipStream_t st = reinterpret_cast<hipStream_t>(stream);
  DevParams d;
  rc = to_dev(params, &d);
  if (rc) return rc;
  if (bound && (sh.gen_tab || sh.HB > 4))
    return fail(NAIS_E_UNSUPPORTED, "nais_pair_table_bound: native embed widths with hidden <= 128 only");
  if (one && (params->variant != NAIS_VARIANT_BASIC || (sh.DH != 16 && sh.DH != 32) || sh.HB > 2))
    return fail(NAIS_E_UNSUPPORTED,
                "nais_pair_table_bound1_queued: NAIS_basic, embed_dim 32 or 64, hidden <= 64");
  if (sh.gen_tab)
    return nais_gx_catalog(params, nullptr, nullptr, nullptr, 0, items, num_items, col0, cols,
                           region_of, coords, latlon_mat, nullptr, 0, nullptr, e, es, ld, st, split);
  const int precision = bound ? NAIS_PRECISION_FP16X3 : params->precision;
  TableOut tab;
  if (split || bound) tab.sel_e = NAIS_SEL_HI;
  if (split) tab.ex = 1;
  tab.ld = ld;
  tab.cols = cols;
  tab.gi = PAIR_GROUP_ITEMS;
  tab.work = work;
  const int64_t groups_per_launch = 65535;
  for (int64_t g0 = 0; g0 * tab.gi < num_items; g0 += groups_per_launch) {
    const int64_t base = g0 * tab.gi;
    tab.nitems = std::min<int64_t>(num_items - base, groups_per_launch * tab.gi);
    tab.e = e + base * ld;
    tab.es = es ? es + base * ld * (split ? 2 : 1) : nullptr;
    tab.col0 = col0;
    const int ng = (int)((tab.nitems + tab.gi - 1) / tab.gi);
    if (one)
      rc = sh.DH == 16 ? (sh.HB == 1 ? launch_x3b_one<16, 1>(d, items + base, ng, st, tab)
                                     : launch_x3b_one<16, 2>(d, items + base, ng, st, tab))
                       : (sh.HB == 1 ? launch_x3b_one<32, 1>(d, items + base, ng, st, tab)
                                     : launch_x3b_one<32, 2>(d, items + base, ng, st, tab));
    else if (precision == NAIS_PRECISION_FP32)
      NAIS_DISPATCH(launch_catalog, sh.DH, sh.HB, params->variant, d, nullptr, items + base, nullptr,
                    ng, region_of, coords, latlon_mat, nullptr, 0, nullptr, st, tab);
    else if (precision == NAIS_PRECISION_FP16X6 || precision == NAIS_PRECISION_FP16X6_PAIRSPLIT)
      NAIS_DISPATCH(launch_catalog_x6b, sh.DH, sh.HB, params->variant, d, nullptr, items + base,
                    nullptr, ng, region_of, coords, latlon_mat, nullptr, 0, nullptr, st, tab);
    else
      NAIS_DISPATCH(launch_catalog_x3b, sh.DH, sh.HB, params->variant, d, nullptr, items + base,
                    nullptr, ng, region_of, coords, latlon_mat, nullptr, 0, nullptr, st, tab);
    if (rc) return rc;
  }
  return NAIS_OK;
}
}

int32_t nais_pair_table(const nais_params_t* params, const int64_t* items, int64_t num_items,
                        int64_t col0, int64_t cols, const int64_t* region_of,
                        const double* coords, const double* latlon_mat, float* e, float* es,
                        int64_t ld, int32_t* work, void* stream) {
  return pair_table_impl(params, items, num_items, col0, cols, region_of, coords, latlon_mat, e, es,
                         ld, work, stream);
}

int32_t nais_pair_table_split(const nais_params_t* params, const int64_t* items, int64_t num_items,
                              int64_t col0, int64_t cols, const int64_t* region_of,
                              const double* coords, const double* latlon_mat, uint32_t* hi,
                              uint32_t* ex, int64_t ld, int32_t* work, void* stream) {
  return pair_table_impl(params, items, num_items, col0, cols, region_of, coords, latlon_mat,
                         reinterpret_cast<float*>(hi), reinterpret_cast<float*>(ex), ld, work, stream,
                         true);
}

int32_t nais_pair_table_bound(const nais_params_t* params, const int64_t* items, int64_t num_items,
                              int64_t col0, int64_t cols, const int64_t* region_of,
                              const double* coords, const double* latlon_mat, uint32_t* hi,
                              int64_t ld, void* stream) {
  return nais_pair_table_bound_queued(params, items, num_items, col0, cols, region_of, coords,
                                      latlon_mat, hi, ld, nullptr, stream);
}

int32_t nais_pair_table_bound_queued(const nais_params_t* params, const int64_t* items,
                                     int64_t num_items, int64_t col0, int64_t cols,
                                     const int64_t* region_of, const double* coords,
                                     const double* latlon_mat, uint32_t* hi, int64_t ld,
                                     int32_t* work, void* stream) {
  return pair_table_impl(params, items, num_items, col0, cols, region_of, coords, latlon_mat,
                         reinterpret_cast<float*>(hi), nullptr, ld, work, stream, false, true);
}

int32_t nais_pair_table_bound1_queued(const nais_params_t* params, const int64_t* items,
                                      int64_t num_items, int64_t col0, int64_t cols,
                                      const int64_t* region_of, const double* coords,
                                      const double* latlon_mat, uint32_t* hi, int64_t ld,
                                      int32_t* work, void* stream) {
  return pair_table_impl(params, items, num_items, col0, cols, region_of, coords, latlon_mat,
                         reinterpret_cast<float*>(hi), nullptr, ld, work, stream, false, true, true);
}

int32_t nais_pair_scales(const nais_params_t* params, const int64_t* items, int64_t num_items,
                         int64_t col0, int64_t cols, int64_t block_cols, float* row_scales,
                         float* col_scales, void* stream) {
  Shape sh;
  int rc = validate(params, &sh);
  if (rc) return rc;
  if (params->variant != NAIS_VARIANT_BASIC || params->precision != NAIS_PRECISION_FP16X6 ||
      (params->embed_dim != 32 && params->embed_dim != 64) || params->hidden > 64)
    return fail(NAIS_E_UNSUPPORTED, "nais_pair_scales: NAIS_basic at fp16x6, embed_dim 32 or 64, hidden <= 64");
  if (num_items < 0 || col0 < 0 || cols < 0 || col0 + cols > params->num_pois || block_cols <= 0)
    return fail(NAIS_E_INVALID, "bad item count, column range or block width");
  if (num_items == 0 && cols == 0) return NAIS_OK;
  if ((num_items > 0 && (!items || !row_scales)) || (cols > 0 && !col_scales))
    return fail(NAIS_E_INVALID, "missing pointer");
  DevParams d;
  rc = to_dev(params, &d);
  if (rc) return rc;
  const int64_t nchunks = (num_items + 31) / 32;
  const int64_t ntiles = (cols + block_cols - 1) / block_cols * ((block_cols + 31) / 32);
  if (nchunks + ntiles > 0x7FFFFFFFll) return fail(NAIS_E_UNSUPPORTED, "too many rows or columns");
  hipStream_t st = reinterpret_cast<hipStream_t>(stream);
  if (params->embed_dim == 32)
    hipLaunchKernelGGL(pair_scales_kernel<32>, dim3((unsigned)(nchunks + ntiles)), dim3(64), 0, st, d, items,
                       num_items, col0, cols, block_cols, nchunks, row_scales, col_scales);
  else
    hipLaunchKernelGGL(pair_scales_kernel<64>, dim3((unsigned)(nchunks + ntiles)), dim3(64), 0, st, d, items,
                       num_items, col0, cols, block_cols, nchunks, row_scales, col_scales);
  return check_launch("pair_scales_kernel");
}

int32_t nais_score_catalog(const nais_params_t* params, const int64_t* indptr,
                           const int64_t* indices, const int32_t* users, int32_t num_users,
                           const int64_t* region_of, const double* coords,
                           const double* latlon_mat, float* scores, int64_t score_ld,
                           int32_t* nan_count, void* stream) {
  Shape sh;
  int rc = validate(params, &sh);
  if (rc) return rc;
  if (num_users < 0) return fail(NAIS_E_INVALID, "num_users < 0");
  if (num_users == 0) return NAIS_OK;
  if (!indptr || !indices || !users || !scores) return fail(NAIS_E_INVALID, "missing pointer");
  if (score_ld < params->num_pois) return fail(NAIS_E_INVALID, "score_ld < num_pois");
  if ((params->variant == NAIS_VARIANT_REGION || params->variant == NAIS_VARIANT_REGION_DISTANCE) &&
      !region_of)
    return fail(NAIS_E_INVALID, "region variants need region_of");
  if ((params->variant == NAIS_VARIANT_REGION_DISTANCE || params->variant == NAIS_VARIANT_DISTANCE) &&
      !coords && !latlon_mat)
    return fail(NAIS_E_INVALID, "region_distance needs coords or latlon_mat");
  hipStream_t st = reinterpret_cast<hipStream_t>(stream);
  DevParams d;
  rc = to_dev(params, &d);
  if (rc) return rc;
  for (int32_t u0 = 0; u0 < num_users; u0 += 65535) {
    const int nb = std::min<int32_t>(65535, num_users - u0);
    if (sh.gen_cat)
      rc = nais_gx_catalog(params, indptr, indices, users + u0, nb, nullptr, 0, 0, 0, region_of,
                           coords, latlon_mat, scores + (int64_t)u0 * score_ld, score_ld, nan_count,
                           nullptr, nullptr, 0, st);
    else if (params->precision == NAIS_PRECISION_FP16X6)
      NAIS_DISPATCH(launch_catalog_x6b, sh.DH, sh.HB, params->variant, d, indptr, indices, users + u0,
                    nb, region_of, coords, latlon_mat, scores + (int64_t)u0 * score_ld, score_ld,
                    nan_count, st);
    else if (params->precision == NAIS_PRECISION_FP16X6_PAIRSPLIT)
      NAIS_DISPATCH(launch_catalog_x6, sh.DH, sh.HB, params->variant, d, indptr, indices, users + u0,
                    nb, region_of, coords, latlon_mat, scores + (int64_t)u0 * score_ld, score_ld,
                    nan_count, st);
    else if (params->precision == NAIS_PRECISION_FP16X3)
      NAIS_DISPATCH(launch_catalog_x3b, sh.DH, sh.HB, params->variant, d, indptr, indices, users + u0,
                    nb, region_of, coords, latlon_mat, scores + (int64_t)u0 * score_ld, score_ld,
                    nan_count, st);
    else if (params->precision == NAIS_PRECISION_FP16X3_PAIRSPLIT)
      NAIS_DISPATCH(launch_catalog_x3, sh.DH, sh.HB, params->variant, d, indptr, indices, users + u0,
                    nb, region_of, coords, latlon_mat, scores + (int64_t)u0 * score_ld, score_ld,
                    nan_count, st);
    else
      NAIS_DISPATCH(launch_catalog, sh.DH, sh.HB, params->variant, d, indptr, indices, users + u0, nb,
                    region_of, coords, latlon_mat, scores + (int64_t)u0 * score_ld, score_ld,
                    nan_count, st);
    if (rc) return rc;
  }
  return NAIS_OK;
// ... 129 lines not shown
```

### poi_recommendation_models_amd/csrc/nais_pairs.hip

```cpp
#include <hip/hip_runtime.h>

#include <math.h>
#include <stdint.h>

#include <algorithm>
#include <string>

#include "nais.h"
#include "nais_internal.h"
#include "nais_geo.h"
#include "nais_fp16x6.h"

namespace {

constexpr int CPL = 4;
typedef float nfv __attribute__((ext_vector_type(CPL)));
typedef double ndv __attribute__((ext_vector_type(CPL)));

__device__ __forceinline__ nfv loadv(const float* p) { return *reinterpret_cast<const nfv*>(p); }

constexpr int SCAN_THREADS = 1024;

__global__ void mark_kernel(const int64_t* __restrict__ indptr, const int64_t* __restrict__ indices,
                            const int32_t* __restrict__ users, int32_t* __restrict__ flag) {
// ... 390 lines not shown
        }
      }
    }
    if (all_zero) continue;
    for (; jj < jn; ++jj) {
      const ndv rv = load_cols<ndv>(pr + bcast64(mlo, mhi, jj) + x, nv);
#pragma unroll
      for (int q = 0; q < CPL; ++q) g[q] = __dmul_rn(g[q], rv[q]);
    }
    if (zero_exit) {
      bool nz = false;
#pragma unroll
      for (int q = 0; q < CPL; ++q) nz |= g[q] != 0.0;
      all_zero = __ballot(nz) == 0ull;
    }
  }
  wave_lds_sync();
  double m = -1.0;
#pragma unroll
  for (int q = 0; q < CPL; ++q) {
    const int64_t xr = x + q;
    if (xr < cols) {
      const int64_t r = xr - s0;
      const bool hist = (hm[w][r >> 5] >> (r & 31)) & 1u;
      const double v = hist ? -1.0 : g[q];
      G[slot * g_ld + (col0 - g_col0) + xr] = v;
      m = fmax(m, v);
    }
  }
#pragma unroll
  for (int o = 32; o > 0; o >>= 1) m = fmax(m, __shfl_xor(m, o));
  if (lane == 0 && m >= 0.0) atomicMax(gmax + slot, (unsigned long long)__double_as_longlong(m));
}

#ifndef NAIS_PAIRS_BGU
#define NAIS_PAIRS_BGU 4
#endif
constexpr int BGU = NAIS_PAIRS_BGU;
constexpr int BCPL = 8;
constexpr int BSTRIPE = 64 * BCPL;
constexpr int BK_LDS = 512;

typedef float f2v __attribute__((ext_vector_type(2)));

__device__ __forceinline__ void bound_rows(const uint32_t* __restrict__ HI, int64_t ld, int32_t mrow,
                                           int jn, uint32_t colbytes, uint32_t voff, f2v (&S)[BCPL / 2],
                                           f2v (&N)[BCPL / 2], float (&A)[BCPL]) {
  auto row = [&](int jj) __attribute__((always_inline)) {
    const int64_t r = __builtin_amdgcn_readlane(mrow, jj);
    return __builtin_amdgcn_make_buffer_rsrc(const_cast<uint32_t*>(HI) + r * ld, (short)0, (int)colbytes,
                                             0x00020000);
  };
  auto acc = [&](const uint4 (&v)[2]) __attribute__((always_inline)) {
    const uint32_t w[BCPL] = {v[0].x, v[0].y, v[0].z, v[0].w, v[1].x, v[1].y, v[1].z, v[1].w};
#pragma unroll
    for (int q = 0; q < BCPL; q += 2) {
      S[q / 2] += f2v{__uint_as_float(w[q] << 16), __uint_as_float(w[q + 1] << 16)};
      N[q / 2] += f2v{__uint_as_float(w[q]), __uint_as_float(w[q + 1])};
      A[q] += fabsf(__uint_as_float(w[q]));
      A[q + 1] += fabsf(__uint_as_float(w[q + 1]));
    }
  };
  auto ld2 = [&](__amdgpu_buffer_rsrc_t rs, uint4 (&v)[2]) __attribute__((always_inline)) {
    const auto a = __builtin_amdgcn_raw_buffer_load_b128(rs, (int)voff, 0, 0);
    const auto b = __builtin_amdgcn_raw_buffer_load_b128(rs, (int)voff + 16, 0, 0);
    v[0] = uint4{a[0], a[1], a[2], a[3]};
    v[1] = uint4{b[0], b[1], b[2], b[3]};
  };
  int jj = 0;
  for (; jj + BGU <= jn; jj += BGU) {
    uint4 v[BGU][2];
#pragma unroll
    for (int g = 0; g < BGU; ++g) ld2(row(jj + g), v[g]);
#pragma unroll
    for (int g = 0; g < BGU; ++g) acc(v[g]);
  }
  for (; jj < jn; ++jj) {
    uint4 v[2];
    ld2(row(jj), v);
    acc(v);
  }
}

__device__ __forceinline__ float sigmoid_ref(float l) { return 1.0f / (1.0f + expf(-l)); }
__device__ __forceinline__ unsigned long long score_key(float sc, int64_t c) {
  return ((unsigned long long)ord_f32_p(sc) << 32) | (unsigned long long)(0xFFFFFFFFu - (uint32_t)c);
}
constexpr unsigned long long KEY_SCORE_MAX = 0xFFFFFFFF00000000ull;

struct Bounds {
  float slo, shi, nlo, nhi, dlo, dhi;
  bool ok;
};
struct Widen {
  float eta, eta2, ds;
};
__device__ __forceinline__ Widen load_widen(const float* __restrict__ widen) {
  Widen w{0.f, 0.f, 0.f};
  if (widen) {
    w.eta = widen[0];
    w.ds = widen[1];
    w.eta2 = w.eta > 0.f ? w.eta * 1.02f + 0x1p-21f : 0.f;
  }
  return w;
}
__device__ __forceinline__ Bounds make_bounds(float S, float N, float A, int64_t hl, float beta,
                                              const Widen& w) {
  Bounds b;
  const float g = (float)hl * 0x1p-23f + 0x1p-20f;
  const float tiny = (float)hl * 0x1p-126f;
  b.slo = S * (1.f - 3.f * g) * (1.f - w.eta);
  b.shi = S * (1.f + 0x1p-7f) * (1.f + 3.f * g) * (1.f + w.eta) + tiny;
  const float rn = (0x1p-7f + 4.f * g + w.eta2) * A + (tiny + S * (1.f + 0x1p-7f) * (1.f + w.eta) * w.ds);
  b.nlo = N - rn;
  b.nhi = N + rn;
  if (beta == 0.5f) {
    b.dlo = sqrtf(b.slo);
    b.dhi = sqrtf(b.shi);
  } else {
    const float p0 = powf(b.slo, beta), p1 = powf(b.shi, beta);
    b.dlo = fminf(p0, p1);
    b.dhi = fmaxf(p0, p1);
  }
  b.ok = b.slo > 0.f && b.dlo > 0.f && __builtin_isfinite(b.dhi) && __builtin_isfinite(b.nlo) &&
         __builtin_isfinite(b.nhi);
  return b;
}
__device__ __forceinline__ float upper_score(const Bounds& b) {
  float l = b.nhi >= 0.f ? b.nhi / b.dlo : b.nhi / b.dhi;
  l += fabsf(l) * 0x1p-19f;
  return fminf(sigmoid_ref(l) * (1.f + 0x1p-20f), 1.0f);
}
__device__ __forceinline__ float lower_score(const Bounds& b) {
  float l = b.nlo >= 0.f ? b.nlo / b.dhi : b.nlo / b.dlo;
  l -= fabsf(l) * 0x1p-19f;
  return l >= 17.f ? 1.0f : sigmoid_ref(l) * (1.f - 0x1p-20f);
}

__device__ __forceinline__ bool may_reach(float S, float N, float A, int64_t hl, float L, const Widen& w) {
  const float g = (float)hl * 0x1p-23f + 0x1p-20f;
  const float tiny = (float)hl * 0x1p-126f;
  const float nhi = N + ((0x1p-7f + 4.f * g + w.eta2) * A + (tiny + S * (1.f + 0x1p-7f) * (1.f + w.eta) * w.ds));
  const float sd = nhi >= 0.f ? S * (1.f - 3.f * g) * (1.f - w.eta)
                              : S * (1.f + 0x1p-7f) * (1.f + 3.f * g) * (1.f + w.eta) + tiny;
  float l = nhi * __builtin_amdgcn_rcpf(__builtin_amdgcn_sqrtf(sd));
  l += fabsf(l) * 0x1p-17f;
  return !(l < L);
}
__device__ __forceinline__ float lthr_of(unsigned long long thr, float beta) {
  if (thr == 0ull || beta != 0.5f) return -__builtin_inff();
  const float ts = unord_f32_p((uint32_t)(thr >> 32));
  if (!(ts > 0.f && ts <= 1.f)) return -__builtin_inff();
  const double p = (double)ts * (1.0 - 0x1p-18);
  double L = log(p / (1.0 - p));
  L -= 1e-6 * (1.0 + fabs(L));
  return (float)L;
}

__device__ void wave_sort_desc(unsigned long long* L, int n) {
  const int lane = threadIdx.x & 63;
  int n2 = 64;
  while (n2 < n) n2 <<= 1;
  for (int i = n + lane; i < n2; i += 64) L[i] = 0ull;
  wave_lds_sync();
  for (int size = 2; size <= n2; size <<= 1) {
    for (int stride = size >> 1; stride > 0; stride >>= 1) {
      for (int i = lane; i < n2; i += 64) {
        const int partner = i ^ stride;
        if (partner > i) {
          const bool desc = (i & size) == 0;
          const unsigned long long a = L[i], b = L[partner];
          if (desc ? (a < b) : (a > b)) {
            L[i] = b;
            L[partner] = a;
          }
        }
      }
      wave_lds_sync();
    }
  }
}

template <int NQ>
__device__ int wave_merge_keys(unsigned long long* L, int cnt, const unsigned long long (&kq)[NQ],
                               uint32_t offer, int k) {
  const int lane = threadIdx.x & 63;
  const int mine_n = __popc(offer);
  int excl = mine_n;
#pragma unroll
  for (int o = 1; o < 64; o <<= 1) {
    const int y = __shfl_up(excl, o);
    if (lane >= o) excl += y;
  }
  const int m = __shfl(excl, 63);
  excl -= mine_n;
  if (m == 0) return cnt;
  int pos = cnt + excl;
#pragma unroll
  for (int q = 0; q < NQ; ++q)
    if ((offer >> q) & 1u) L[pos++] = kq[q];
  const int n = cnt + m;
  wave_sort_desc(L, n);
  return n < k ? n : k;
}

__global__ void __launch_bounds__(GW * 64)
pair_bound_topk_kernel(const uint32_t* __restrict__ HI, int64_t ld, const int32_t* __restrict__ rowmap,
                       const int64_t* __restrict__ indptr, const int64_t* __restrict__ indices,
                       const int32_t* __restrict__ users, int32_t nusers, int64_t col0, int64_t cols,
                       float beta, int k, unsigned long long* __restrict__ lokeys,
                       int32_t* __restrict__ locount, unsigned long long* __restrict__ surv,
                       int32_t* __restrict__ scount, int cap, const int32_t* __restrict__ erows,
                       const int64_t* __restrict__ spans, int32_t* __restrict__ work,
                       const float* __restrict__ widen) {
  __shared__ unsigned long long lk[GW][BK_LDS];
  __shared__ uint32_t hm[GW][BSTRIPE / 32];
  const int lane = threadIdx.x & 63, w = __builtin_amdgcn_readfirstlane(threadIdx.x >> 6);
  constexpr int GQ = 4;
  const Widen wd = load_widen(widen);
  int64_t qnext = 0, qend = 0;
  for (int64_t it = 0;; ++it) {
  int64_t slot;
  if (work) {
    if (qnext == qend) {
      int got = 0;
      if (lane == 0) got = atomicAdd(work, GQ);
      qnext = __builtin_amdgcn_readfirstlane(got);
      qend = qnext + GQ;
    }
    slot = qnext++;
  } else {
    if (it > 0) break;
    slot = int64_t(blockIdx.x) * GW + w;
  }
  if (slot >= nusers) break;
  int64_t hb, hl;
  if (spans) {
    hb = spans[2 * slot];
    hl = spans[2 * slot + 1];
  } else {
    const int64_t u = users[slot];
    hb = indptr[u];
    hl = indptr[u + 1] - hb;
  }
  const int cnt = locount[slot];
  const unsigned long long lk_last = lokeys[slot * k + k - 1];
  int sc = scount[slot];
  const int64_t x = int64_t(lane) * BCPL;
  if (lane < BSTRIPE / 32) hm[w][lane] = 0u;
  wave_lds_sync();
  f2v S2[BCPL / 2], N2[BCPL / 2];
  float A[BCPL];
#pragma unroll
  for (int q = 0; q < BCPL / 2; ++q) S2[q] = N2[q] = f2v{0.f, 0.f};
#pragma unroll
  for (int q = 0; q < BCPL; ++q) A[q] = 0.f;
  for (int64_t j0 = 0; j0 < hl; j0 += 64) {
    const int jn = __builtin_amdgcn_readfirstlane((int)std::min<int64_t>(64, hl - j0));
    int32_t mrow = 0;
    if (lane < jn) {
      const int64_t e = hb + j0 + lane;
      const int64_t c = indices[e];
      mrow = erows ? erows[e] : rowmap[c];
      const int64_t r = c - col0;
      if (r >= 0 && r < cols) atomicOr(&hm[w][r >> 5], 1u << (r & 31));
    }
    bound_rows(HI, ld, mrow, jn, (uint32_t)(cols * 4), (uint32_t)(x * 4), S2, N2, A);
  }
  wave_lds_sync();
  float S[BCPL], N[BCPL];
#pragma unroll
  for (int q = 0; q < BCPL; ++q) {
    S[q] = S2[q / 2][q & 1];
    N[q] = N2[q / 2][q & 1];
  }
  const unsigned long long thr = cnt == k ? lk_last : 0ull;
  uint32_t ho[BCPL], lo_[BCPL];
  uint32_t live = 0, offer = 0;
  const uint32_t idb0 = 0xFFFFFFFFu - (uint32_t)(col0 + x);
  auto key_of = [&](uint32_t ord, int q) __attribute__((always_inline)) {
    return ((unsigned long long)ord << 32) | (unsigned long long)(idb0 - (uint32_t)q);
  };
  const float Lthr = lthr_of(thr, beta);
#pragma unroll
  for (int q = 0; q < BCPL; ++q) {
    ho[q] = 0u;
    lo_[q] = 0u;
    const int64_t r = x + q;
    if (r < cols && !((hm[w][r >> 5] >> (r & 31)) & 1u)) {
      if (hl == 0) {
        live |= 1u << q;
        ho[q] = lo_[q] = ord_f32_p(0.5f);
      } else if (may_reach(S[q], N[q], A[q], hl, Lthr, wd)) {
        live |= 1u << q;
        const Bounds b = make_bounds(S[q], N[q], A[q], hl, beta, wd);
        ho[q] = b.ok ? ord_f32_p(upper_score(b)) : 0xFFFFFFFFu;
        if (b.ok && key_of(ho[q], q) > thr) lo_[q] = ord_f32_p(lower_score(b));
      }
      if (lo_[q] != 0u && key_of(lo_[q], q) > thr) offer |= 1u << q;
    }
  }
  unsigned long long* L = lk[w];
  int nk = cnt;
  const bool merged = __ballot(offer != 0u) != 0ull;
  if (merged) {
    for (int i = lane; i < cnt; i += 64) L[i] = lokeys[slot * k + i];
    wave_lds_sync();
    const unsigned long long l0[4] = {key_of(lo_[0], 0), key_of(lo_[1], 1), key_of(lo_[2], 2), key_of(lo_[3], 3)};
    const unsigned long long l1[4] = {key_of(lo_[4], 4), key_of(lo_[5], 5), key_of(lo_[6], 6), key_of(lo_[7], 7)};
    nk = wave_merge_keys<4>(L, nk, l0, offer & 0xFu, k);
    nk = wave_merge_keys<4>(L, nk, l1, offer >> 4, k);
    for (int i = lane; i < nk; i += 64) lokeys[slot * k + i] = L[i];
    if (lane == 0) locount[slot] = nk;
  }
  const unsigned long long tau = nk == k ? (merged ? L[k - 1] : thr) : 0ull;
  uint32_t sv = 0;
#pragma unroll
  for (int q = 0; q < BCPL; ++q)
    if (((live >> q) & 1u) && key_of(ho[q], q) >= tau) sv |= 1u << q;
  const int mine_n = __popc(sv);
  int excl = mine_n;
#pragma unroll
  for (int o = 1; o < 64; o <<= 1) {
    const int y = __shfl_up(excl, o);
    if (lane >= o) excl += y;
  }
  const int m = __shfl(excl, 63);
  excl -= mine_n;
  if (m > 0 && sc >= 0) {
    unsigned long long* list = surv + slot * (int64_t)cap;
    if (sc + m > cap) {
      int wpos = 0;
      for (int i0 = 0; i0 < sc; i0 += 64) {
        const bool in = i0 + lane < sc;
        const unsigned long long v = in ? list[i0 + lane] : 0ull;
        const bool keep = in && v >= tau;
        const unsigned long long bal = __ballot(keep);
        const int before = __popcll(bal & ((1ull << lane) - 1ull));
        if (keep) list[wpos + before] = v;
        wpos += __popcll(bal);
      }
      sc = wpos + m > cap ? -1 : wpos;
    }
    if (sc >= 0) {
      int pos = sc + excl;
#pragma unroll
      for (int q = 0; q < BCPL; ++q)
        if ((sv >> q) & 1u) list[pos++] = key_of(ho[q], q);
      sc += m;
    }
    if (lane == 0) scount[slot] = sc;
  }
  wave_lds_sync();
  }
}

constexpr int RF_LDS = 512;
constexpr int RF_CAND = 512;

__global__ void __launch_bounds__(GW * 64)
pair_refine_topk_kernel(const uint2* __restrict__ X, int64_t bstride, int64_t ld,
                        int64_t bcols, const int32_t* __restrict__ rowmap,
                        const int64_t* __restrict__ indptr, const int64_t* __restrict__ indices,
                        const int32_t* __restrict__ users, int32_t nusers, int64_t col0, int64_t cols,
                        float beta, int k, const unsigned long long* __restrict__ lokeys,
                        const int32_t* __restrict__ locount, const unsigned long long* __restrict__ surv,
                        const int32_t* __restrict__ scount, int cap,
                        const unsigned long long* __restrict__ tau_in, unsigned long long* __restrict__ keys,
                        int32_t* __restrict__ kcount, int32_t* __restrict__ nan_count,
                        int32_t* __restrict__ stats, const int32_t* __restrict__ erows) {
  __shared__ unsigned long long lk[GW][RF_LDS];
  __shared__ uint32_t cb[GW][128];
  __shared__ unsigned long long ck[GW][RF_CAND];
  const int lane = threadIdx.x & 63, w = __builtin_amdgcn_readfirstlane(threadIdx.x >> 6);
  const int64_t slot = int64_t(blockIdx.x) * GW + w;
  if (slot >= nusers) return;
  const int64_t u = users[slot];
  const int64_t hb = indptr[u], hl = indptr[u + 1] - hb;
  const int cnt = locount[slot];
  unsigned long long tau = cnt == k ? lokeys[slot * k + k - 1] : 0ull;
  if (tau_in && tau_in[slot] > tau) tau = tau_in[slot];
  const int sc = scount[slot];
  unsigned long long* L = lk[w];
  int nk = 0;
  int nan = 0, refined = 0;
  auto batch = [&](int64_t r, bool valid) __attribute__((always_inline)) {
    const int64_t rr = valid ? r : 0;
    const int64_t b = rr / bcols;
    const int64_t xo = b * bstride + (rr - b * bcols);
    const int64_t c = col0 + rr;
    float Sa = 0.f, Na = 0.f;
    bool in_hist = false;
    for (int64_t j0 = 0; j0 < hl; j0 += 64) {
      const int jn = __builtin_amdgcn_readfirstlane((int)std::min<int64_t>(64, hl - j0));
      int64_t mine = 0, mid = -1;
      if (lane < jn) {
        mid = indices[hb + j0 + lane];
        mine = int64_t(erows ? erows[hb + j0 + lane] : rowmap[mid]) * ld;
      }
      const uint32_t mlo = uint32_t(mine), mhi = uint32_t(mine >> 32);
      const uint32_t ilo = uint32_t(mid), ihi = uint32_t(mid >> 32);
      int jj = 0;
      for (; jj + GU <= jn; jj += GU) {
        uint2 v[GU];
        int64_t id[GU];
#pragma unroll
        for (int g = 0; g < GU; ++g) {
          id[g] = bcast64(ilo, ihi, jj + g);
          v[g] = X[bcast64(mlo, mhi, jj + g) + xo];
        }
#pragma unroll
        for (int g = 0; g < GU; ++g) {
          Sa += __uint_as_float(v[g].x);
          Na += __uint_as_float(v[g].y);
          in_hist |= id[g] == c;
        }
      }
      for (; jj < jn; ++jj) {
        const uint2 v = X[bcast64(mlo, mhi, jj) + xo];
        Sa += __uint_as_float(v.x);
        Na += __uint_as_float(v.y);
        in_hist |= bcast64(ilo, ihi, jj) == c;
      }
    }
    unsigned long long kq[1] = {0ull};
    uint32_t offer = 0;
    if (valid && !in_hist) {
      float logit = 0.f;
      if (hl > 0) logit = Na / ((beta == 0.5f) ? sqrtf(Sa) : powf(Sa, beta));
      float s = 1.0f / (1.0f + expf(-logit));
      if (logit != logit) {
        s = __builtin_nanf("");
        ++nan;
      }
      kq[0] = score_key(s, c);
      ++refined;
      const unsigned long long lthr = nk == k ? L[k - 1] : 0ull;
// ... 479 lines not shown
  if (num_users == 0 || cols == 0) return NAIS_OK;
  if (!e || !es || !rowmap || !indptr || !indices || !users || !scores)
    return nais_internal_fail(NAIS_E_INVALID, "missing pointer");
  if (ld % 4 != 0) return nais_internal_fail(NAIS_E_INVALID, "ld must be a multiple of 4");
  hipStream_t st = reinterpret_cast<hipStream_t>(stream);
  const int64_t stripes = (cols + STRIPE - 1) / STRIPE;
  if (stripes > 65535) return nais_internal_fail(NAIS_E_UNSUPPORTED, "cols > 65535 * 256");
  hipLaunchKernelGGL(pair_gather_kernel, dim3((unsigned)((num_users + GW - 1) / GW), (unsigned)stripes),
                     dim3(GW * 64), 0, st, e, es, ld, rowmap, indptr, indices, users, num_users, col0,
                     cols, beta, scores, score_ld, score_col0, nan_count);
  return nais_internal_check_launch("pair_gather_kernel");
}

int32_t nais_pair_gather_topk(const float* e, const float* es, int64_t ld, const int32_t* rowmap,
                              const int64_t* indptr, const int64_t* indices, const int32_t* users,
                              int32_t num_users, int64_t col0, int64_t cols, float beta, int32_t k,
                              uint64_t* keys, int32_t* kcount, int32_t* nan_count, int32_t* work,
                              void* stream) {
  if (num_users < 0 || col0 < 0 || cols < 0 || ld < cols || k <= 0)
    return nais_internal_fail(NAIS_E_INVALID, "bad shape");
  if (k > TK_LDS - STRIPE) return nais_internal_fail(NAIS_E_UNSUPPORTED, "k must be <= 256");
  if (col0 + cols > 0xFFFFFFFFll) return nais_internal_fail(NAIS_E_UNSUPPORTED, "POI ids must fit 32 bits");
  if (num_users == 0 || cols == 0) return NAIS_OK;
  if (!e || !es || !rowmap || !indptr || !indices || !users || !keys || !kcount)
    return nais_internal_fail(NAIS_E_INVALID, "missing pointer");
  if (ld % 4 != 0) return nais_internal_fail(NAIS_E_INVALID, "ld must be a multiple of 4");
  hipStream_t st = reinterpret_cast<hipStream_t>(stream);
  unsigned groups = (unsigned)((num_users + GW - 1) / GW);
  if (work) {
    const int ncu = nais_internal_stream_cus(st);
    if (ncu <= 0) return nais_internal_fail(NAIS_E_HIP, "device attributes");
    groups = std::min<unsigned>(groups, (unsigned)ncu * 5u);
  }
  for (int64_t s0 = 0; s0 < cols; s0 += STRIPE) {
    if (work && hipMemsetAsync(work, 0, sizeof(int32_t), st) != hipSuccess)
      return nais_internal_fail(NAIS_E_HIP, "hipMemsetAsync(work)");
    hipLaunchKernelGGL(pair_gather_topk_kernel, dim3(groups), dim3(GW * 64), 0, st, e + s0, es + s0, ld,
                       rowmap, indptr, indices, users, num_users, col0 + s0,
                       std::min<int64_t>(STRIPE, cols - s0), beta, (int)k,
                       reinterpret_cast<unsigned long long*>(keys), kcount, nan_count, work);
    const int32_t rc = nais_internal_check_launch("pair_gather_topk_kernel");
    if (rc) return rc;
  }
  return NAIS_OK;
}

int32_t nais_pair_bound_topk_widened(const uint32_t* hi, int64_t ld, const int32_t* rowmap,
                                     const int64_t* indptr, const int64_t* indices, const int32_t* users,
                                     int32_t num_users, int64_t col0, int64_t cols, float beta, int32_t k,
                                     uint64_t* lo_keys, int32_t* lo_count, uint64_t* surv,
                                     int32_t* surv_count, int32_t surv_cap, const int32_t* entry_rows,
                                     const int64_t* spans, const float* widen, int32_t* work,
                                     void* stream) {
  if (num_users < 0 || col0 < 0 || cols < 0 || ld < cols || k <= 0 || surv_cap < 64)
    return nais_internal_fail(NAIS_E_INVALID, "bad shape");
  if (k > BK_LDS - 256) return nais_internal_fail(NAIS_E_UNSUPPORTED, "k must be <= 256");
  if (col0 + cols > 0xFFFFFFFFll) return nais_internal_fail(NAIS_E_UNSUPPORTED, "POI ids must fit 32 bits");
  if (num_users == 0 || cols == 0) return NAIS_OK;
  if (!hi || !rowmap || !indptr || !indices || !users || !lo_keys || !lo_count || !surv || !surv_count)
    return nais_internal_fail(NAIS_E_INVALID, "missing pointer");
  if (ld % 4 != 0 || (reinterpret_cast<uintptr_t>(hi) & 15) != 0)
    return nais_internal_fail(NAIS_E_INVALID, "ld must be a multiple of 4 and hi 16-byte aligned");
  hipStream_t st = reinterpret_cast<hipStream_t>(stream);
  unsigned groups = (unsigned)((num_users + GW - 1) / GW);
  if (work) {
    const int ncu = nais_internal_stream_cus(st);
    if (ncu <= 0) return nais_internal_fail(NAIS_E_HIP, "device attributes");
    groups = std::min<unsigned>(groups, (unsigned)ncu * 5u);
  }
  for (int64_t s0 = 0; s0 < cols; s0 += BSTRIPE) {
    if (work && hipMemsetAsync(work, 0, sizeof(int32_t), st) != hipSuccess)
      return nais_internal_fail(NAIS_E_HIP, "hipMemsetAsync(work)");
    hipLaunchKernelGGL(pair_bound_topk_kernel, dim3(groups), dim3(GW * 64), 0, st, hi + s0, ld, rowmap,
                       indptr, indices, users, num_users, col0 + s0, std::min<int64_t>(BSTRIPE, cols - s0),
                       beta, (int)k, reinterpret_cast<unsigned long long*>(lo_keys), lo_count,
                       reinterpret_cast<unsigned long long*>(surv), surv_count, (int)surv_cap, entry_rows,
                       spans, work, widen);
    const int32_t rc = nais_internal_check_launch("pair_bound_topk_kernel");
    if (rc) return rc;
  }
  return NAIS_OK;
}

int32_t nais_pair_bound_topk(const uint32_t* hi, int64_t ld, const int32_t* rowmap,
                             const int64_t* indptr, const int64_t* indices, const int32_t* users,
                             int32_t num_users, int64_t col0, int64_t cols, float beta, int32_t k,
                             uint64_t* lo_keys, int32_t* lo_count, uint64_t* surv, int32_t* surv_count,
                             int32_t surv_cap, const int32_t* entry_rows, const int64_t* spans,
                             int32_t* work, void* stream) {
  return nais_pair_bound_topk_widened(hi, ld, rowmap, indptr, indices, users, num_users, col0, cols, beta,
                                      k, lo_keys, lo_count, surv, surv_count, surv_cap, entry_rows, spans,
                                      nullptr, work, stream);
}

int32_t nais_pair_refine_topk(const uint32_t* ex, int64_t block_stride,
                              int64_t ld, int64_t block_cols, const int32_t* rowmap,
                              const int64_t* indptr, const int64_t* indices, const int32_t* users,
                              int32_t num_users, int64_t col0, int64_t cols, float beta, int32_t k,
                              const uint64_t* lo_keys, const int32_t* lo_count, const uint64_t* surv,
                              const int32_t* surv_count, int32_t surv_cap, const uint64_t* tau,
                              uint64_t* keys, int32_t* kcount, int32_t* nan_count, int32_t* stats,
                              const int32_t* entry_rows, void* stream) {
  if (num_users < 0 || col0 < 0 || cols < 0 || k <= 0 || surv_cap < 64 || block_cols <= 0 ||
      ld < std::min<int64_t>(block_cols, cols) || block_stride < 0 || block_stride % 2 != 0)
    return nais_internal_fail(NAIS_E_INVALID, "bad shape");
  if (k > RF_LDS - 256) return nais_internal_fail(NAIS_E_UNSUPPORTED, "k must be <= 256");
  if (col0 + cols > 0xFFFFFFFFll) return nais_internal_fail(NAIS_E_UNSUPPORTED, "POI ids must fit 32 bits");
  if (num_users == 0) return NAIS_OK;
  if (!rowmap || !indptr || !indices || !users || !lo_keys || !lo_count || !surv || !surv_count ||
      !keys || !kcount || (cols > 0 && !ex))
    return nais_internal_fail(NAIS_E_INVALID, "missing pointer");
  hipLaunchKernelGGL(pair_refine_topk_kernel, dim3((unsigned)((num_users + GW - 1) / GW)), dim3(GW * 64), 0,
                     reinterpret_cast<hipStream_t>(stream), reinterpret_cast<const uint2*>(ex), block_stride / 2, ld,
                     block_cols,
                     rowmap, indptr, indices, users, num_users, col0, cols, beta, (int)k,
                     reinterpret_cast<const unsigned long long*>(lo_keys), lo_count,
                     reinterpret_cast<const unsigned long long*>(surv), surv_count, (int)surv_cap,
                     reinterpret_cast<const unsigned long long*>(tau),
                     reinterpret_cast<unsigned long long*>(keys), kcount, nan_count, stats, entry_rows);
  return nais_internal_check_launch("pair_refine_topk_kernel");
}

namespace {
int exact_model(const nais_params_t* p, ExactModel* md, int* D, int* MB) {
  if (!p) return nais_internal_fail(NAIS_E_INVALID, "params is NULL");
  if (p->variant != NAIS_VARIANT_BASIC || p->precision != NAIS_PRECISION_FP16X6 ||
      (p->embed_dim != 32 && p->embed_dim != 64) || p->hidden <= 0 || p->hidden > 64 ||
      p->item_dim != p->embed_dim || p->din != p->embed_dim)
    return nais_internal_fail(NAIS_E_UNSUPPORTED,
                              "exact refine: NAIS_basic at fp16x6, embed_dim 32 or 64, hidden <= 64");
  if (!p->embed_history || !p->embed_target || !p->w1 || !p->b1 || !p->w2)
    return nais_internal_fail(NAIS_E_INVALID, "missing parameter pointer");
  *md = ExactModel{p->embed_history, p->embed_target, p->w1, p->b1, p->w2, p->hidden};
  *D = p->embed_dim;
  *MB = p->hidden <= 32 ? 2 : 4;
  return NAIS_OK;
}
}

int32_t nais_pair_refine_topk_exact(const nais_params_t* params, const float* row_scales,
                                    const float* col_scales, const int32_t* rowmap, const int64_t* indptr,
                                    const int64_t* indices, const int32_t* users, int32_t num_users,
                                    int64_t col0, int64_t cols, int32_t k, const uint64_t* lo_keys,
                                    const int32_t* lo_count, const uint64_t* surv, const int32_t* surv_count,
                                    int32_t surv_cap, const uint64_t* tau, uint64_t* keys, int32_t* kcount,
                                    int32_t* nan_count, int32_t* stats, const int32_t* entry_rows,
                                    void* stream) {
  ExactModel md;
  int D, MB;
  const int rc = exact_model(params, &md, &D, &MB);
  if (rc) return rc;
  if (num_users < 0 || col0 < 0 || cols < 0 || k <= 0 || surv_cap < 64 || col0 + cols > params->num_pois)
    return nais_internal_fail(NAIS_E_INVALID, "bad shape");
  if (k > RF_LDS - 256) return nais_internal_fail(NAIS_E_UNSUPPORTED, "k must be <= 256");
  if (col0 + cols > 0x7FFFFFFFll) return nais_internal_fail(NAIS_E_UNSUPPORTED, "POI ids must fit 31 bits");
  if (num_users == 0) return NAIS_OK;
  if (!rowmap || !indptr || !indices || !users || !lo_keys || !lo_count || !surv || !surv_count ||
      !keys || !kcount || !row_scales || (cols > 0 && !col_scales))
    return nais_internal_fail(NAIS_E_INVALID, "missing pointer");
  const dim3 grid((unsigned)((num_users + GW - 1) / GW)), block(GW * 64);
  hipStream_t st = reinterpret_cast<hipStream_t>(stream);
#define NAIS_EXACT_REFINE(D_, MB_)                                                                   \
  hipLaunchKernelGGL((pair_refine_exact_kernel<D_, MB_>), grid, block, 0, st, md, row_scales,        \
                     col_scales, rowmap, indptr, indices, users, num_users, col0, cols, params->beta, \
                     (int)k, reinterpret_cast<const unsigned long long*>(lo_keys), lo_count,          \
                     reinterpret_cast<const unsigned long long*>(surv), surv_count, (int)surv_cap,    \
// ... 113 lines not shown
```

Before: 16.11 billion.

## Quantize one-product bound table to 8-bit pairs with shared 16-column scales

```diff
diff --git a/include/nais.h b/include/nais.h
--- a/include/nais.h
+++ b/include/nais.h
@@ -8,7 +8,7 @@
 extern "C" {
 #endif
 
-#define NAIS_ABI_VERSION 19
+#define NAIS_ABI_VERSION 20
 
 #define NAIS_VARIANT_BASIC 0
 #define NAIS_VARIANT_REGION 1
@@ -136,6 +136,18 @@
                               const int32_t* surv_count, int32_t surv_cap, const uint64_t* tau,
                               uint64_t* keys, int32_t* kcount, int32_t* nan_count, int32_t* stats,
                               const int32_t* entry_rows, void* stream);
+int64_t nais_q16_pitch(int64_t ld);
+int32_t nais_pair_table_bound1_q16_queued(const nais_params_t* params, const int64_t* items,
+                                          int64_t num_items, int64_t col0, int64_t cols,
+                                          const int64_t* region_of, const double* coords,
+                                          const double* latlon_mat, void* q16, int64_t ld,
+                                          int64_t pitch, int32_t* work, void* stream);
+int32_t nais_pair_bound_topk_q16(const void* q16, int64_t ld, int64_t pitch, const int32_t* rowmap,
+                                 const int64_t* indptr, const int64_t* indices, const int32_t* users,
+                                 int32_t num_users, int64_t col0, int64_t cols, float beta, int32_t k,
+                                 uint64_t* lo_keys, int32_t* lo_count, uint64_t* surv,
+                                 int32_t* surv_count, int32_t surv_cap, const int32_t* entry_rows,
+                                 const int64_t* spans, const float* widen, int32_t* work, void* stream);
 int32_t nais_pair_table_bound(const nais_params_t* params, const int64_t* items, int64_t num_items,
                               int64_t col0, int64_t cols, const int64_t* region_of,
                               const double* coords, const double* latlon_mat, uint32_t* hi,
diff --git a/poi_recommendation_models_amd/_capi.py b/poi_recommendation_models_amd/_capi.py
--- a/poi_recommendation_models_amd/_capi.py
+++ b/poi_recommendation_models_amd/_capi.py
@@ -7,7 +7,7 @@
 LIB_NAME = "libnais_hip.so"
 LIB_PATH = os.path.join(HERE, LIB_NAME)
 
-ABI_VERSION = 19
+ABI_VERSION = 20
 PRECISION_FP32, PRECISION_FP16X3, PRECISION_FP16X3_PAIRSPLIT = 0, 1, 2
 PRIOR_FINITE = 1
 PRECISION_FP16X6, PRECISION_FP16X6_PAIRSPLIT = 3, 4
@@ -31,6 +31,7 @@
            "nais_pair_bound_topk", "nais_pair_refine_topk", "nais_pair_table_bound",
            "nais_pair_bound_topk_widened", "nais_pair_scales", "nais_pair_refine_topk_exact",
            "nais_pair_recompute", "nais_pair_table_bound_queued", "nais_pair_table_bound1_queued",
+           "nais_q16_pitch", "nais_pair_table_bound1_q16_queued", "nais_pair_bound_topk_q16",
            "nais_geoie_table", "nais_geoie_score", "nais_geoie_forward",
            "nais_geoie_make_train_batch", "nais_geoie_train_step_workspace_size",
            "nais_geoie_train_step", "nais_sgd")
@@ -245,6 +246,14 @@
     lib.nais_pair_bound_topk_widened.restype = i32
     lib.nais_pair_bound_topk_widened.argtypes = [vp, i64, vp, vp, vp, vp, i32, i64, i64, f32, i32, vp, vp,
                                                  vp, vp, i32, vp, vp, vp, vp, vp]
+    lib.nais_q16_pitch.restype = i64
+    lib.nais_q16_pitch.argtypes = [i64]
+    lib.nais_pair_table_bound1_q16_queued.restype = i32
+    lib.nais_pair_table_bound1_q16_queued.argtypes = [ctypes.POINTER(NaisParams), vp, i64, i64, i64, vp,
+                                                      vp, vp, vp, i64, i64, vp, vp]
+    lib.nais_pair_bound_topk_q16.restype = i32
+    lib.nais_pair_bound_topk_q16.argtypes = [vp, i64, i64, vp, vp, vp, vp, i32, i64, i64, f32, i32, vp,
+                                             vp, vp, vp, i32, vp, vp, vp, vp, vp]
     lib.nais_pair_scales.restype = i32
     lib.nais_pair_scales.argtypes = [ctypes.POINTER(NaisParams), vp, i64, i64, i64, i64, vp, vp, vp]
     lib.nais_pair_refine_topk_exact.restype = i32
diff --git a/poi_recommendation_models_amd/catalog.py b/poi_recommendation_models_amd/catalog.py
--- a/poi_recommendation_models_amd/catalog.py
+++ b/poi_recommendation_models_amd/catalog.py
@@ -198,21 +198,24 @@
 X3Q_GATHER_MARGIN = 1.14
 X1Q_RATE = 6.0e14
 X1Q_GATHER_MARGIN = 1.34
+X1Q16_RATE = 5.7e14
+X1Q16_GATHER_MARGIN = 1.16
 PAIR_BOUNDED = True
 PAIR_ONDEMAND_REFINE = os.environ.get("NAIS_PAIR_ONDEMAND_REFINE", "1") != "0"
 PAIR_ONDEMAND_ETA_MAX = 2.0 ** -9
 PAIR_ONDEMAND_ONE_PRODUCT = os.environ.get("NAIS_PAIR_ONDEMAND_ONE_PRODUCT", "1") != "0"
 PAIR_ONDEMAND_ETA1_MAX = 2.0 ** -7
+PAIR_BOUND_Q16 = os.environ.get("NAIS_PAIR_BOUND_Q16", "1") != "0"
 PAIR_SURV_CAP = 1024
 PAIR_SHORT_CHAINS = os.environ.get("NAIS_PAIR_SHORT_CHAINS", "1") != "0"
 PAIR_BOUNDED_STRIPE = 512
 _masked: dict = {}
 
 
-def bounded_gather_cu_seconds(entries, NC, users, k):
+def bounded_gather_cu_seconds(entries, NC, users, k, bytes_per_pair=4.0):
     launches = np.ceil(NC / PAIR_BOUNDED_STRIPE)
     ins = k * (1.0 + np.log(max(float(NC), float(k)) / k))
-    return entries * NC * 4.0 / 90.4e9 + 512e-9 * users * launches + 68e-9 * users * ins
+    return entries * NC * bytes_per_pair / 90.4e9 + 512e-9 * users * launches + 68e-9 * users * ins
 
 
 def ondemand_widening(model, products=3):
@@ -272,7 +275,7 @@
 
 
 def auto_table_cus(model, J, NC, entries, ncu, prior=False, block_bytes=None, work_queues=True,
-                   gather_bytes=8, k=None, users=None, products=None, table_queue=False):
+                   gather_bytes=8, k=None, users=None, products=None, table_queue=False, q16=False):
     H, din = model.attn_layer1.weight.shape
     prec = getattr(model, "precision", "fp16x6")
     given = products
@@ -299,6 +302,10 @@
     t_tab = J * NC * 2.0 * H * din_k * products / (1.3e14 if products == 1 else rate)
     if x1q:
         t_tab = J * NC * 2.0 * H * din_k / X1Q_RATE
+    q16 = bool(q16) and x1q
+    if q16:
+        t_tab = J * NC * 2.0 * H * din_k / X1Q16_RATE
+        gbytes = entries * NC * 2.25
     if x6n and dist:
         t_tab *= 1.0 + 16.0 / (3.0 * D)
     if prior:
@@ -312,8 +319,12 @@
             per_cu = gbytes / bounded_gather_cu_seconds(entries, NC, users, k)
         if x3q:
             per_cu /= X3Q_GATHER_MARGIN
-        if x1q:
+        if x1q and not q16:
             per_cu /= X1Q_GATHER_MARGIN
+        if q16:
+            if users and k:
+                per_cu = gbytes / bounded_gather_cu_seconds(entries, NC, users, k, 2.25)
+            per_cu /= X1Q16_GATHER_MARGIN
     cap = 7.5e12
     best, best_t = ncu // 2, None
     for n in range((ncu // 4 + step - 1) // step * step, ncu - step + 1, step):
@@ -449,6 +460,8 @@
         pri_coords = torch.as_tensor(np.ascontiguousarray(pc, dtype=np.float64)).to(dev)
         prior_flags = _capi.PRIOR_FINITE if _prior_entries_finite(pa, pb) else 0
     pr_of = {}
+    q16 = [False]
+    qpitch = [0]
 
     wq_slots = torch.zeros(8, dtype=torch.int32, device=dev) if PAIR_WORK_QUEUE else None
     wq_of = {}
@@ -466,6 +479,12 @@
 
     def table(tab, c0, w, stream_):
         if isinstance(tab, tuple) and len(tab) == 1:
+            if ond_products == 1 and q16[0]:
+                _capi.check(lib.nais_pair_table_bound1_q16_queued(
+                    prm, items.data_ptr(), J, c0, w, _capi.ptr(reg), _capi.ptr(cor), _capi.ptr(llm),
+                    tab[0].data_ptr(), ld, qpitch[0], wq(stream_), stream_),
+                    "nais_pair_table_bound1_q16_queued")
+                return
             if ond_products == 1:
                 _capi.check(lib.nais_pair_table_bound1_queued(
                     prm, items.data_ptr(), J, c0, w, _capi.ptr(reg), _capi.ptr(cor), _capi.ptr(llm),
@@ -520,6 +539,15 @@
                 b = m if b is None else b
                 if b <= a:
                     return
+                if bnd[0] and q16[0]:
+                    _capi.check(lib.nais_pair_bound_topk_q16(
+                        tab[0].data_ptr(), ld, qpitch[0], rowmap.data_ptr(), csr.indptr.data_ptr(),
+                        csr.indices.data_ptr(), u_dev.data_ptr() + 4 * a, b - a, c0, w, float(model.beta), k,
+                        lokeys.data_ptr() + 8 * k * a, locount.data_ptr() + 4 * a,
+                        surv.data_ptr() + 8 * PAIR_SURV_CAP * a, scount.data_ptr() + 4 * a, PAIR_SURV_CAP,
+                        _capi.ptr(erows), spans.data_ptr() + 16 * a if spans is not None else None,
+                        ond.data_ptr(), wq(stream_), stream_), "nais_pair_bound_topk_q16")
+                    return
                 if bnd[0]:
                     _capi.check(lib.nais_pair_bound_topk_widened(
                         tab[0].data_ptr(), ld, rowmap.data_ptr(), csr.indptr.data_ptr(), csr.indices.data_ptr(),
@@ -568,12 +596,19 @@
                 if ond is not None:
                     ondm[0] = bool(agree_min(int(ondm[0]), dev, tau_group))
             bnd[0] = bnd[0] or ondm[0]
+            q16[0] = ondm[0] and ond_products == 1 and PAIR_BOUND_Q16
+            qpitch[0] = int(lib.nais_q16_pitch(ld)) if q16[0] else 0
             if events is not None:
                 events.append(("pair_route", None, None, "ondemand" if ondm[0] else
                                ("split16" if bnd[0] else "exact")))
+                if ondm[0]:
+                    events.append(("ondemand_words", None, None, "q16" if q16[0] else "hi"))
             if bnd[0]:
+                if q16[0]:
+                    ring = [torch.empty(J, qpitch[0], dtype=torch.uint8, device=dev) for _ in range(nring)]
+                elif ondm[0]:
+                    ring = [torch.empty(J, ld, dtype=torch.int32, device=dev) for _ in range(nring)]
                 if ondm[0]:
-                    ring = [torch.empty(J, ld, dtype=torch.int32, device=dev) for _ in range(nring)]
                     ring_done = [None] * nring
                     rowsc = torch.empty(max(J, 1), 2, dtype=torch.float32, device=dev)
                     colsc = torch.empty(NC, dtype=torch.float32, device=dev)
@@ -600,7 +635,7 @@
                                         J * ld * (4 if ondm[0] else 8),
                                         work_queues=wq_both, gather_bytes=4 if bnd[0] else 8, k=k,
                                         users=m, products=ond_products if ondm[0] else None,
-                                        table_queue=ondm[0])
+                                        table_queue=ondm[0], q16=q16[0])
                          if PAIR_TABLE_CUS < 0 else PAIR_TABLE_CUS)
             wq_on[0] = table_cus % max(1, ncu // 8) != 0 or (ondm[0] and wq_both)
             if events is not None:
diff --git a/poi_recommendation_models_amd/csrc/nais_kernels.hip b/poi_recommendation_models_amd/csrc/nais_kernels.hip
--- a/poi_recommendation_models_amd/csrc/nais_kernels.hip
+++ b/poi_recommendation_models_amd/csrc/nais_kernels.hip
@@ -49,6 +49,8 @@
   int32_t ngroups = 0, ntiles = 0;
   uint32_t sel_e = NAIS_SEL_E;
   int32_t ex = 0;
+  int64_t qpitch = 0;
+  int32_t qpairs = 0;
 };
 __device__ __forceinline__ void tab_put(const TableOut& t, int64_t row, int64_t x, float e, float es) {
   const int64_t o = row * t.ld + x;
@@ -469,6 +471,37 @@
     c = mfma16(a[0], b[0], c);
   }
   return c;
+}
+
+struct Q16Words {
+  uint32_t pair, scale;
+};
+__device__ __forceinline__ uint32_t q16_row_max(uint32_t v) {
+#define NAIS_ROR_MAX(n) \
+  v = max(v, (uint32_t)__builtin_amdgcn_update_dpp(0, (int)v, 0x120 + (n), 0xF, 0xF, false))
+  NAIS_ROR_MAX(8);
+  NAIS_ROR_MAX(4);
+  NAIS_ROR_MAX(2);
+  NAIS_ROR_MAX(1);
+#undef NAIS_ROR_MAX
+  return v;
+}
+__device__ __forceinline__ Q16Words q16_words(float e, float p, bool valid, int hh) {
+  constexpr float C255 = (float)((1.0 + 0x1p-7) * (1.0 + 0x1p-13) / 255.0);
+  constexpr float C127 = (float)((1.0 + 0x1p-7) * (1.0 + 0x1p-13) / 127.0);
+  const float x = hh ? p : e;
+  const uint32_t M = q16_row_max(valid ? (__float_as_uint(x) & 0x7FFFFFFFu) : 0u);
+  uint32_t qb = __float_as_uint(__uint_as_float(M) * (hh ? C127 : C255)) & 0xFFFF0000u;
+  qb = max(qb, 0x0D800000u);
+  qb = M ? qb : 0u;
+  const float r = M ? __builtin_amdgcn_rcpf(__uint_as_float(qb)) : 0.f;
+  const float u = __builtin_amdgcn_fmed3f(fmaf(x, r, hh ? 128.f : 0.f), 0.f, 255.f);
+  const uint32_t pk = qb | (uint32_t)u;
+  const auto sw = __builtin_amdgcn_permlane32_swap(pk, pk, false, false);
+  Q16Words w;
+  w.pair = __builtin_amdgcn_perm(sw[1], sw[0], 0x0C0C0400u);
+  w.scale = __builtin_amdgcn_perm(sw[1], sw[0], NAIS_SEL_HI);
+  return w;
 }
 
 __device__ __forceinline__ float2 lane_halves(float v) {
@@ -817,7 +850,7 @@
   static_assert(!PIPE || G % 2 == 0, "the pipelined steps alternate two accumulator sets per item");
 };
 
-template <int DH, int HB, int VAR, int NW, int NPC, bool QUEUE = false, bool ONE = false>
+template <int DH, int HB, int VAR, int NW, int NPC, bool QUEUE = false, bool ONE = false, bool Q16 = false>
 __global__ void __launch_bounds__(NW * 64, NW >= 8 ? 1 : 8 / NW)
 catalog_score_x3b_kernel(DevParams p, const int64_t* __restrict__ indptr,
                          const int64_t* __restrict__ indices, const int32_t* __restrict__ users,
@@ -833,6 +866,7 @@
   constexpr bool PIPE = C::PIPE;
   static_assert(!ONE || (NPC == 2 && PIPE && !DIST),
                 "one-product logits: the pipelined fp16x3 shapes, no distance inputs");
+  static_assert(!Q16 || ONE, "q16 words: the one-product bound table only");
   constexpr bool SMF = JCB == 32;
   extern __shared__ __attribute__((aligned(16))) char smem[];
   uint4* ring = reinterpret_cast<uint4*>(smem);
@@ -1011,6 +1045,18 @@
     }
     const bool keep = hid[pj] != (int32_t)c;
     const float e = expf(a) * (keep ? 1.f : 0.f);
+    if constexpr (Q16) {
+      if (live) {
+        const Q16Words qw = q16_words(e, e * sv, valid, hh);
+        if (valid && hh == 0) {
+          const int64_t x = c - tab.col0;
+          char* row = reinterpret_cast<char*>(tab.e) + (hbeg + j0 + pj) * tab.qpitch;
+          reinterpret_cast<uint16_t*>(row + tab.qpairs)[x] = (uint16_t)qw.pair;
+          if ((lane & 15) == 0) reinterpret_cast<uint32_t*>(row)[x >> 4] = qw.scale;
+        }
+      }
+      return;
+    }
     if (live) {
       if (tab.e) {
         if (valid && hh == 0) {
@@ -2552,13 +2598,13 @@
   }
 }
 
-template <int DH, int HB>
+template <int DH, int HB, bool Q16 = false>
 int launch_x3b_one(const DevParams& d, const int64_t* indices, int ng, hipStream_t stream,
                    const TableOut& tab) {
   constexpr int NW = WAVES, VAR = NAIS_VARIANT_BASIC;
   const size_t lds = CfgB<DH, HB, false, NW, 2, 1>::BYTES;
-  auto kern = catalog_score_x3b_kernel<DH, HB, VAR, NW, 2, false, true>;
-  auto kq = catalog_score_x3b_kernel<DH, HB, VAR, NW, 2, true, true>;
+  auto kern = catalog_score_x3b_kernel<DH, HB, VAR, NW, 2, false, true, Q16>;
+  auto kq = catalog_score_x3b_kernel<DH, HB, VAR, NW, 2, true, true, Q16>;
   static bool attr_set = false;
   if (!attr_set) {
     (void)hipFuncSetAttribute(reinterpret_cast<const void*>(kern),
@@ -2812,7 +2858,8 @@
 int32_t pair_table_impl(const nais_params_t* params, const int64_t* items, int64_t num_items,
                         int64_t col0, int64_t cols, const int64_t* region_of, const double* coords,
                         const double* latlon_mat, float* e, float* es, int64_t ld, int32_t* work,
-                        void* stream, bool split = false, bool bound = false, bool one = false) {
+                        void* stream, bool split = false, bool bound = false, bool one = false,
+                        int64_t qpitch = 0) {
   Shape sh;
   int rc = validate(params, &sh);
   if (rc) return rc;
@@ -2821,6 +2868,9 @@
   if (num_items == 0 || cols == 0) return NAIS_OK;
   if (!items || !e || (!es && !bound)) return fail(NAIS_E_INVALID, "missing pointer");
   if (ld < cols) return fail(NAIS_E_INVALID, "ld < cols");
+  if (qpitch && (!one || ld > (1 << 24) || qpitch != nais_q16_pitch(ld) ||
+                 (reinterpret_cast<uintptr_t>(e) & 3) != 0))
+    return fail(NAIS_E_INVALID, "q16: pitch must be nais_q16_pitch(ld) and the block 4-byte aligned");
   if ((params->variant == NAIS_VARIANT_REGION || params->variant == NAIS_VARIANT_REGION_DISTANCE) &&
       !region_of)
     return fail(NAIS_E_INVALID, "region variants need region_of");
@@ -2855,7 +2905,15 @@
     tab.es = es ? es + base * ld * (split ? 2 : 1) : nullptr;
     tab.col0 = col0;
     const int ng = (int)((tab.nitems + tab.gi - 1) / tab.gi);
-    if (one)
+    if (qpitch) {
+      tab.e = reinterpret_cast<float*>(reinterpret_cast<char*>(e) + base * qpitch);
+      tab.qpitch = qpitch;
+      tab.qpairs = (int32_t)(4 * ((ld + 15) / 16));
+      rc = sh.DH == 16 ? (sh.HB == 1 ? launch_x3b_one<16, 1, true>(d, items + base, ng, st, tab)
+                                     : launch_x3b_one<16, 2, true>(d, items + base, ng, st, tab))
+                       : (sh.HB == 1 ? launch_x3b_one<32, 1, true>(d, items + base, ng, st, tab)
+                                     : launch_x3b_one<32, 2, true>(d, items + base, ng, st, tab));
+    } else if (one)
       rc = sh.DH == 16 ? (sh.HB == 1 ? launch_x3b_one<16, 1>(d, items + base, ng, st, tab)
                                      : launch_x3b_one<16, 2>(d, items + base, ng, st, tab))
                        : (sh.HB == 1 ? launch_x3b_one<32, 1>(d, items + base, ng, st, tab)
@@ -2916,6 +2974,17 @@
                                       int32_t* work, void* stream) {
   return pair_table_impl(params, items, num_items, col0, cols, region_of, coords, latlon_mat,
                          reinterpret_cast<float*>(hi), nullptr, ld, work, stream, false, true, true);
+}
+
+int32_t nais_pair_table_bound1_q16_queued(const nais_params_t* params, const int64_t* items,
+                                          int64_t num_items, int64_t col0, int64_t cols,
+                                          const int64_t* region_of, const double* coords,
+                                          const double* latlon_mat, void* q16, int64_t ld,
+                                          int64_t pitch, int32_t* work, void* stream) {
+  if (pitch <= 0) return fail(NAIS_E_INVALID, "q16: pitch must be nais_q16_pitch(ld)");
+  return pair_table_impl(params, items, num_items, col0, cols, region_of, coords, latlon_mat,
+                         reinterpret_cast<float*>(q16), nullptr, ld, work, stream, false, true, true,
+                         pitch);
 }
 
 int32_t nais_pair_scales(const nais_params_t* params, const int64_t* items, int64_t num_items,
diff --git a/poi_recommendation_models_amd/csrc/nais_pairs.hip b/poi_recommendation_models_amd/csrc/nais_pairs.hip
--- a/poi_recommendation_models_amd/csrc/nais_pairs.hip
+++ b/poi_recommendation_models_amd/csrc/nais_pairs.hip
@@ -496,6 +496,64 @@
   }
 }
 
+constexpr int BGU8 = 2 * BGU;
+#ifndef NAIS_Q16_COLA
+#define NAIS_Q16_COLA 0
+#endif
+constexpr int QNA = NAIS_Q16_COLA ? BCPL : 1;
+#ifndef NAIS_Q16_WAVES
+#define NAIS_Q16_WAVES 4
+#endif
+__device__ __forceinline__ void bound_rows_q16(const uint32_t* __restrict__ Q, int64_t pitch4, int32_t mrow,
+                                               int jn, uint32_t recbytes, uint32_t voff, uint32_t soff,
+                                               f2v (&S)[BCPL / 2], f2v (&N)[BCPL / 2], f2v& QQ,
+                                               float (&A)[QNA]) {
+  auto row = [&](int jj) __attribute__((always_inline)) {
+    const int64_t r = __builtin_amdgcn_readlane(mrow, jj);
+    return __builtin_amdgcn_make_buffer_rsrc(const_cast<uint32_t*>(Q) + r * pitch4, (short)0,
+                                             (int)((recbytes + 3u) & ~3u), 0x00020000);
+  };
+  struct Row {
+    uint4 w;
+    uint32_t s;
+  };
+  auto ldr = [&](__amdgpu_buffer_rsrc_t rs, Row& v) __attribute__((always_inline)) {
+    const auto a = __builtin_amdgcn_raw_buffer_load_b128(rs, (int)voff, 0, 0);
+    v.w = uint4{a[0], a[1], a[2], a[3]};
+    v.s = __builtin_amdgcn_raw_buffer_load_b32(rs, (int)soff, 0, 0);
+  };
+  auto acc = [&](const Row& v) __attribute__((always_inline)) {
+    const float qe = __uint_as_float(v.s << 16), qs = __uint_as_float(v.s & 0xFFFF0000u);
+    QQ += f2v{qe, qs};
+    const f2v qe2{qe, qe}, qs2{qs, qs};
+    const uint32_t w[BCPL / 2] = {v.w.x, v.w.y, v.w.z, v.w.w};
+#pragma unroll
+    for (int q = 0; q < BCPL / 2; ++q) {
+      const f2v me{(float)(w[q] & 0xFFu), (float)((w[q] >> 16) & 0xFFu)};
+      const f2v ms{(float)((w[q] >> 8) & 0xFFu), (float)(w[q] >> 24)};
+      S[q] = __builtin_elementwise_fma(me, qe2, S[q]);
+      N[q] = __builtin_elementwise_fma(ms, qs2, N[q]);
+      if constexpr (NAIS_Q16_COLA) {
+        A[(2 * q) % QNA] = fmaf(fabsf(ms[0] - 128.f), qs, A[(2 * q) % QNA]);
+        A[(2 * q + 1) % QNA] = fmaf(fabsf(ms[1] - 128.f), qs, A[(2 * q + 1) % QNA]);
+      }
+    }
+  };
+  int jj = 0;
+  for (; jj + BGU8 <= jn; jj += BGU8) {
+    Row v[BGU8];
+#pragma unroll
+    for (int g = 0; g < BGU8; ++g) ldr(row(jj + g), v[g]);
+#pragma unroll
+    for (int g = 0; g < BGU8; ++g) acc(v[g]);
+  }
+  for (; jj < jn; ++jj) {
+    Row v;
+    ldr(row(jj), v);
+    acc(v);
+  }
+}
+
 __device__ __forceinline__ float sigmoid_ref(float l) { return 1.0f / (1.0f + expf(-l)); }
 __device__ __forceinline__ unsigned long long score_key(float sc, int64_t c) {
   return ((unsigned long long)ord_f32_p(sc) << 32) | (unsigned long long)(0xFFFFFFFFu - (uint32_t)c);
@@ -569,6 +627,52 @@
   double L = log(p / (1.0 - p));
   L -= 1e-6 * (1.0 + fabs(L));
   return (float)L;
+}
+
+struct QEnds {
+  float slo, shi, nlo, nhi;
+};
+__device__ __forceinline__ QEnds q16_ends(float S, float N, float Qe, float Qs, float Acol, int64_t hl,
+                                          const Widen& w) {
+  const float g = (float)hl * 0x1p-23f + 0x1p-20f;
+  const float tiny = (float)hl * 0x1p-126f;
+  const float A = NAIS_Q16_COLA ? (Acol + Qs) * (1.f + 0x1p-10f) : 128.f * (1.f + 0x1p-10f) * Qs;
+  const float su = S + (1.f + 0x1p-13f) * Qe;
+  QEnds q;
+  q.slo = (S - 0x1p-13f * Qe) * (1.f - 3.f * g) * (1.f - w.eta);
+  q.shi = su * (1.f + 3.f * g) * (1.f + w.eta) + tiny;
+  const float rn = (4.f * g + w.eta2) * A + (tiny + su * (1.f + 0x1p-7f) * (1.f + w.eta) * w.ds);
+  q.nlo = N - 512.f * g * Qs - rn;
+  q.nhi = N + (1.f + 512.f * g) * Qs + rn;
+  return q;
+}
+__device__ __forceinline__ Bounds make_bounds_q16(float S, float N, float Qe, float Qs, float Acol,
+                                                  int64_t hl, float beta, const Widen& w) {
+  const QEnds q = q16_ends(S, N, Qe, Qs, Acol, hl, w);
+  Bounds b;
+  b.slo = q.slo;
+  b.shi = q.shi;
+  b.nlo = q.nlo;
+  b.nhi = q.nhi;
+  if (beta == 0.5f) {
+    b.dlo = sqrtf(b.slo);
+    b.dhi = sqrtf(b.shi);
+  } else {
+    const float p0 = powf(b.slo, beta), p1 = powf(b.shi, beta);
+    b.dlo = fminf(p0, p1);
+    b.dhi = fmaxf(p0, p1);
+  }
+  b.ok = b.slo > 0.f && b.dlo > 0.f && __builtin_isfinite(b.dhi) && __builtin_isfinite(b.nlo) &&
+         __builtin_isfinite(b.nhi);
+  return b;
+}
+__device__ __forceinline__ bool may_reach_q16(float S, float N, float Qe, float Qs, float Acol, int64_t hl,
+                                              float L, const Widen& w) {
+  const QEnds q = q16_ends(S, N, Qe, Qs, Acol, hl, w);
+  const float sd = q.nhi >= 0.f ? q.slo : q.shi;
+  float l = q.nhi * __builtin_amdgcn_rcpf(__builtin_amdgcn_sqrtf(sd));
+  l += fabsf(l) * 0x1p-17f;
+  return !(l < L) || !(q.slo > 0.f);
 }
 
 __device__ void wave_sort_desc(unsigned long long* L, int n) {
@@ -618,15 +722,17 @@
   return n < k ? n : k;
 }
 
-__global__ void __launch_bounds__(GW * 64)
-pair_bound_topk_kernel(const uint32_t* __restrict__ HI, int64_t ld, const int32_t* __restrict__ rowmap,
-                       const int64_t* __restrict__ indptr, const int64_t* __restrict__ indices,
-                       const int32_t* __restrict__ users, int32_t nusers, int64_t col0, int64_t cols,
-                       float beta, int k, unsigned long long* __restrict__ lokeys,
-                       int32_t* __restrict__ locount, unsigned long long* __restrict__ surv,
-                       int32_t* __restrict__ scount, int cap, const int32_t* __restrict__ erows,
-                       const int64_t* __restrict__ spans, int32_t* __restrict__ work,
-                       const float* __restrict__ widen) {
+template <bool Q16>
+__device__ __forceinline__ void
+pair_bound_topk_body(const uint32_t* __restrict__ HI, int64_t ld, uint32_t qpairs, uint32_t qx0,
+                     const int32_t* __restrict__ rowmap,
+                     const int64_t* __restrict__ indptr, const int64_t* __restrict__ indices,
+                     const int32_t* __restrict__ users, int32_t nusers, int64_t col0, int64_t cols,
+                     float beta, int k, unsigned long long* __restrict__ lokeys,
+                     int32_t* __restrict__ locount, unsigned long long* __restrict__ surv,
+                     int32_t* __restrict__ scount, int cap, const int32_t* __restrict__ erows,
+                     const int64_t* __restrict__ spans, int32_t* __restrict__ work,
+                     const float* __restrict__ widen) {
   __shared__ unsigned long long lk[GW][BK_LDS];
   __shared__ uint32_t hm[GW][BSTRIPE / 32];
   const int lane = threadIdx.x & 63, w = __builtin_amdgcn_readfirstlane(threadIdx.x >> 6);
@@ -664,11 +770,12 @@
   if (lane < BSTRIPE / 32) hm[w][lane] = 0u;
   wave_lds_sync();
   f2v S2[BCPL / 2], N2[BCPL / 2];
-  float A[BCPL];
+  float A[Q16 ? QNA : BCPL];
+  f2v QQ{0.f, 0.f};
 #pragma unroll
   for (int q = 0; q < BCPL / 2; ++q) S2[q] = N2[q] = f2v{0.f, 0.f};
 #pragma unroll
-  for (int q = 0; q < BCPL; ++q) A[q] = 0.f;
+  for (int q = 0; q < (Q16 ? QNA : BCPL); ++q) A[q] = 0.f;
   for (int64_t j0 = 0; j0 < hl; j0 += 64) {
     const int jn = __builtin_amdgcn_readfirstlane((int)std::min<int64_t>(64, hl - j0));
     int32_t mrow = 0;
@@ -679,7 +786,11 @@
       const int64_t r = c - col0;
       if (r >= 0 && r < cols) atomicOr(&hm[w][r >> 5], 1u << (r & 31));
     }
-    bound_rows(HI, ld, mrow, jn, (uint32_t)(cols * 4), (uint32_t)(x * 4), S2, N2, A);
+    if constexpr (Q16)
+      bound_rows_q16(HI, ld, mrow, jn, qpairs + 2u * (qx0 + (uint32_t)cols), qpairs + 2u * (qx0 + (uint32_t)x),
+                     4u * ((qx0 >> 4) + (uint32_t)(lane >> 1)), S2, N2, QQ, reinterpret_cast<float (&)[QNA]>(A));
+    else
+      bound_rows(HI, ld, mrow, jn, (uint32_t)(cols * 4), (uint32_t)(x * 4), S2, N2, A);
   }
   wave_lds_sync();
   float S[BCPL], N[BCPL];
@@ -687,6 +798,7 @@
   for (int q = 0; q < BCPL; ++q) {
     S[q] = S2[q / 2][q & 1];
     N[q] = N2[q / 2][q & 1];
+    if constexpr (Q16) N[q] = fmaf(-128.f, QQ[1], N[q]);
   }
   const unsigned long long thr = cnt == k ? lk_last : 0ull;
   uint32_t ho[BCPL], lo_[BCPL];
@@ -705,9 +817,11 @@
       if (hl == 0) {
         live |= 1u << q;
         ho[q] = lo_[q] = ord_f32_p(0.5f);
-      } else if (may_reach(S[q], N[q], A[q], hl, Lthr, wd)) {
+      } else if (Q16 ? may_reach_q16(S[q], N[q], QQ[0], QQ[1], A[Q16 ? q % QNA : 0], hl, Lthr, wd)
+                     : may_reach(S[q], N[q], A[Q16 ? 0 : q], hl, Lthr, wd)) {
         live |= 1u << q;
-        const Bounds b = make_bounds(S[q], N[q], A[q], hl, beta, wd);
+        const Bounds b = Q16 ? make_bounds_q16(S[q], N[q], QQ[0], QQ[1], A[Q16 ? q % QNA : 0], hl, beta, wd)
+                             : make_bounds(S[q], N[q], A[Q16 ? 0 : q], hl, beta, wd);
         ho[q] = b.ok ? ord_f32_p(upper_score(b)) : 0xFFFFFFFFu;
         if (b.ok && key_of(ho[q], q) > thr) lo_[q] = ord_f32_p(lower_score(b));
       }
@@ -767,6 +881,32 @@
   }
   wave_lds_sync();
   }
+}
+
+__global__ void __launch_bounds__(GW * 64)
+pair_bound_topk_kernel(const uint32_t* __restrict__ HI, int64_t ld, const int32_t* __restrict__ rowmap,
+                       const int64_t* __restrict__ indptr, const int64_t* __restrict__ indices,
+                       const int32_t* __restrict__ users, int32_t nusers, int64_t col0, int64_t cols,
+                       float beta, int k, unsigned long long* __restrict__ lokeys,
+                       int32_t* __restrict__ locount, unsigned long long* __restrict__ surv,
+                       int32_t* __restrict__ scount, int cap, const int32_t* __restrict__ erows,
+                       const int64_t* __restrict__ spans, int32_t* __restrict__ work,
+                       const float* __restrict__ widen) {
+  pair_bound_topk_body<false>(HI, ld, 0u, 0u, rowmap, indptr, indices, users, nusers, col0, cols, beta, k,
+                              lokeys, locount, surv, scount, cap, erows, spans, work, widen);
+}
+
+__global__ void __launch_bounds__(GW * 64, NAIS_Q16_WAVES)
+pair_bound_topk_q16_kernel(const uint32_t* __restrict__ Q, int64_t pitch4, uint32_t qpairs, uint32_t qx0,
+                           const int32_t* __restrict__ rowmap, const int64_t* __restrict__ indptr,
+                           const int64_t* __restrict__ indices, const int32_t* __restrict__ users,
+                           int32_t nusers, int64_t col0, int64_t cols, float beta, int k,
+                           unsigned long long* __restrict__ lokeys, int32_t* __restrict__ locount,
+                           unsigned long long* __restrict__ surv, int32_t* __restrict__ scount, int cap,
+                           const int32_t* __restrict__ erows, const int64_t* __restrict__ spans,
+                           int32_t* __restrict__ work, const float* __restrict__ widen) {
+  pair_bound_topk_body<true>(Q, pitch4, qpairs, qx0, rowmap, indptr, indices, users, nusers, col0, cols,
+                             beta, k, lokeys, locount, surv, scount, cap, erows, spans, work, widen);
 }
 
 constexpr int RF_LDS = 512;
@@ -1412,6 +1552,48 @@
   return NAIS_OK;
 }
 
+int64_t nais_q16_pitch(int64_t ld) {
+  return ld <= 0 ? 0 : (4 * ((ld + 15) / 16) + 2 * ld + 127) / 128 * 128;
+}
+
+int32_t nais_pair_bound_topk_q16(const void* q16, int64_t ld, int64_t pitch, const int32_t* rowmap,
+                                 const int64_t* indptr, const int64_t* indices, const int32_t* users,
+                                 int32_t num_users, int64_t col0, int64_t cols, float beta, int32_t k,
+                                 uint64_t* lo_keys, int32_t* lo_count, uint64_t* surv,
+                                 int32_t* surv_count, int32_t surv_cap, const int32_t* entry_rows,
+                                 const int64_t* spans, const float* widen, int32_t* work, void* stream) {
+  if (num_users < 0 || col0 < 0 || cols < 0 || ld < cols || k <= 0 || surv_cap < 64)
+    return nais_internal_fail(NAIS_E_INVALID, "bad shape");
+  if (k > BK_LDS - 256) return nais_internal_fail(NAIS_E_UNSUPPORTED, "k must be <= 256");
+  if (col0 + cols > 0xFFFFFFFFll) return nais_internal_fail(NAIS_E_UNSUPPORTED, "POI ids must fit 32 bits");
+  if (num_users == 0 || cols == 0) return NAIS_OK;
+  if (!q16 || !rowmap || !indptr || !indices || !users || !lo_keys || !lo_count || !surv || !surv_count)
+    return nais_internal_fail(NAIS_E_INVALID, "missing pointer");
+  if (ld > (1 << 24) || pitch != nais_q16_pitch(ld) || (reinterpret_cast<uintptr_t>(q16) & 15) != 0)
+    return nais_internal_fail(NAIS_E_INVALID, "pitch must be nais_q16_pitch(ld) and q16 16-byte aligned");
+  hipStream_t st = reinterpret_cast<hipStream_t>(stream);
+  unsigned groups = (unsigned)((num_users + GW - 1) / GW);
+  if (work) {
+    const int ncu = nais_internal_stream_cus(st);
+    if (ncu <= 0) return nais_internal_fail(NAIS_E_HIP, "device attributes");
+    groups = std::min<unsigned>(groups, (unsigned)ncu * 5u);
+  }
+  const uint32_t qpairs = (uint32_t)(4 * ((ld + 15) / 16));
+  for (int64_t s0 = 0; s0 < cols; s0 += BSTRIPE) {
+    if (work && hipMemsetAsync(work, 0, sizeof(int32_t), st) != hipSuccess)
+      return nais_internal_fail(NAIS_E_HIP, "hipMemsetAsync(work)");
+    hipLaunchKernelGGL(pair_bound_topk_q16_kernel, dim3(groups), dim3(GW * 64), 0, st,
+                       reinterpret_cast<const uint32_t*>(q16), pitch / 4, qpairs, (uint32_t)s0, rowmap,
+                       indptr, indices, users, num_users, col0 + s0, std::min<int64_t>(BSTRIPE, cols - s0),
+                       beta, (int)k, reinterpret_cast<unsigned long long*>(lo_keys), lo_count,
+                       reinterpret_cast<unsigned long long*>(surv), surv_count, (int)surv_cap, entry_rows,
+                       spans, work, widen);
+    const int32_t rc = nais_internal_check_launch("pair_bound_topk_q16_kernel");
+    if (rc) return rc;
+  }
+  return NAIS_OK;
+}
+
 int32_t nais_pair_bound_topk(const uint32_t* hi, int64_t ld, const int32_t* rowmap,
                              const int64_t* indptr, const int64_t* indices, const int32_t* users,
                              int32_t num_users, int64_t col0, int64_t cols, float beta, int32_t k,
```

Result: faster. 17.77 billion (median of 6 runs) (+10.4%).
